# rajgandhi1/threecrate

Measured on AMD Instinct MI355X. Metric: ICP iterations/sec (whole job: k=16 normals + 50-iter point-to-plane ICP per 1M-pt pair; tc_cloud handles, inputs resident in HBM), higher is better.
Workload: dtype f32; 1 GPU; 1000000-pt uniform-random cloud, k=16 normals + 50-iter point-to-plane ICP, independent sigma = 0.0001 noise on source and target, correspondences returned (BASELINE configs[1]; one independent pair per GPU); points=1000000, k=16, parallelism=pairs1, interface=tc_cloud handles (one index build per cloud)

## Files before the change

threecrate_amd/csrc/api.hip:

```cpp
#include "tc_internal.h"
#include <sched.h>
#include <time.h>

#include <algorithm>
#include <cmath>
#include <cstdlib>
#include <cstring>
#include <memory>

namespace tc {

[[maybe_unused]] constexpr int kDebugPrintOnlyBits = 8 | 64 | 256 | 1024;
int debug_flags() {
    static const int flags = [] {
        const char *e = getenv("TC_DEBUG");
        const int f = e ? atoi(e) : 0;
#ifdef TC_DEV
        return f;
#else
        return f & kDebugPrintOnlyBits;
#endif
    }();
    return flags;
}
// ... 67 lines not shown
        for (auto &pb : ctx->pool) (void)hipFree(pb.p);
        ctx->pool.clear(); ctx->pool_bytes = 0;
        e = hipMalloc(&b.p, want);
    }
    if (e != hipSuccess) {
        b.p = nullptr;
        return fail(ctx, TC_GPU, std::string("hipMalloc(") + std::to_string(want) + "): " + hipGetErrorString(e));
    }
    b.cap = want;
    return TC_OK;
}

ProfScope::ProfScope(tc_context *c, const char *name, bool dominant) : ctx(c) {
    if (ctx->profiling != 1 && ctx->profiling != 2) return;
    if (ctx->profiling == 2 && (!dominant || (ctx->prof_tick++ % 37u) != 0)) return;
    for (size_t i = 0; i < ctx->timers.size(); ++i)
        if (ctx->timers[i].name == name) { idx = (int)i; break; }
    if (idx < 0) { ctx->timers.push_back(KernelTimer{name, {}, 0, 0.0, 1e300, 0.0}); idx = (int)ctx->timers.size() - 1; }
    auto get = [&]() {
        hipEvent_t e = nullptr;
        if (!ctx->event_pool.empty()) { e = ctx->event_pool.back(); ctx->event_pool.pop_back(); }
        else (void)hipEventCreate(&e);
        return e;
    };
    e0 = get(); e1 = get();
    ext = dominant;
    if (!ext) (void)hipEventRecord(e0, ctx->stream);
}
ProfScope::~ProfScope() {
    if (idx < 0) return;
    if (!ext) (void)hipEventRecord(e1, ctx->stream);
    ctx->timers[idx].pending.emplace_back(e0, e1);
}

bool pinned_poll_enabled() {
    const char *e = getenv("TC_NO_PINNED_POLL");
    return !(e && atoi(e) != 0);
}

void *pinned_dev_ptr(tc_context *ctx, const void *host_addr) {
    if (!ctx->pinned_dev) {
        void *d = nullptr;
        if (hipHostGetDevicePointer(&d, ctx->pinned, 0) != hipSuccess) return nullptr;
        ctx->pinned_dev = d;
    }
    return (char *)ctx->pinned_dev + ((const char *)host_addr - (const char *)ctx->pinned);
}

static inline void cpu_relax() {
#if defined(__x86_64__) || defined(__i386__)
    __builtin_ia32_pause();
#elif defined(__aarch64__)
    asm volatile("yield" ::: "memory");
#else
    sched_yield();
#endif
}

tc_status wait_pinned_word(tc_context *ctx, volatile uint32_t *word, const char *what) {
    struct timespec t0 = {0, 0};
    bool sleeping = false;
    for (unsigned spins = 0; *word == 0u; ++spins) {
        if (sleeping || (spins & 1023u) == 1023u) {
            const hipError_t q = hipStreamQuery(ctx->stream);
            if (q == hipSuccess) { if (*word == 0u) return fail(ctx, TC_GPU, std::string("internal error: ") + what + ": the stream drained without the word being written"); break; }
            if (q != hipErrorNotReady) return fail(ctx, TC_GPU, std::string(what) + ": " + hipGetErrorString(q));
            if (!sleeping && spins >= 4096u) {
                struct timespec t;
                clock_gettime(CLOCK_MONOTONIC, &t);
                if (t0.tv_sec == 0 && t0.tv_nsec == 0) t0 = t;
                sleeping = (t.tv_sec - t0.tv_sec) * 1000000000ll + (t.tv_nsec - t0.tv_nsec) > 2000000ll;
            }
        }
        if (sleeping) { const struct timespec d = {0, 50000}; nanosleep(&d, nullptr); }
        else if (spins > 4096u) sched_yield();
        else cpu_relax();
    }
    __atomic_thread_fence(__ATOMIC_ACQUIRE);
    return TC_OK;
}

void free_buf(DevBuf &b) { if (b.p) (void)hipFree(b.p); b.p = nullptr; b.cap = 0; }

tc_status upload_async(tc_context *ctx, void *d_dst, const void *h_src, size_t bytes) {
    if (bytes < ((size_t)8 << 20)) {
        TC_HIP_TRY(ctx, hipMemcpyAsync(d_dst, h_src, bytes, hipMemcpyHostToDevice, ctx->stream));
        return TC_OK;
    }
    ctx->upload_used_copy_stream = true;
    if (!ctx->copy_stream) TC_HIP_TRY(ctx, hipStreamCreateWithFlags(&ctx->copy_stream, hipStreamNonBlocking));
    if (!ctx->upload_event) TC_HIP_TRY(ctx, hipEventCreateWithFlags(&ctx->upload_event, hipEventDisableTiming));
    TC_HIP_TRY(ctx, hipMemcpyAsync(d_dst, h_src, bytes, hipMemcpyHostToDevice, ctx->copy_stream));
    return TC_OK;
}
tc_status uploads_issued(tc_context *ctx) {
    if (!ctx->upload_used_copy_stream) return TC_OK;
    ctx->upload_used_copy_stream = false;
    TC_HIP_TRY(ctx, hipEventRecord(ctx->upload_event, ctx->copy_stream));
    ctx->upload_pending = true;
    return TC_OK;
}
tc_status wait_uploads(tc_context *ctx) {
    if (!ctx->upload_pending) return TC_OK;
    ctx->upload_pending = false;
    TC_HIP_TRY(ctx, hipStreamWaitEvent(ctx->stream, ctx->upload_event, 0));
    return TC_OK;
}

tc_status stage_in(tc_context *ctx, DevBuf &b, const void *h_src, size_t bytes) {
    if (tc_status s = ensure(ctx, b, bytes)) return s;
    TC_HIP_TRY(ctx, hipMemcpyAsync(b.p, h_src, bytes, hipMemcpyHostToDevice, ctx->stream));
    return TC_OK;
}

tc_status synced(tc_context *ctx) {
    TC_HIP_TRY(ctx, hipStreamSynchronize(ctx->stream));
    return TC_OK;
}
tc_status stage_out(tc_context *ctx, void *h_dst, const void *d_src, size_t bytes) {
    TC_HIP_TRY(ctx, hipMemcpyAsync(h_dst, d_src, bytes, hipMemcpyDeviceToHost, ctx->stream));
    return synced(ctx);
}
tc_status read_back(tc_context *ctx, void *host_dst, const void *dev_src, size_t bytes) {
    if (tc_status s = stage_out(ctx, host_dst, dev_src, bytes)) return s;
    TC_HIP_TRY(ctx, hipGetLastError());
    return TC_OK;
}

float normals_cell_factor(size_t k, bool large) {
    const double K1 = (double)k + 1.0;
    const double lam = K1 + 3.1 * std::sqrt(K1) + 2.0;
    const double c = std::cbrt(lam / 4.18879);
    return (float)((large ? 1.03 : 0.95) * c / 2.0);
}

float normals_target_ppo(size_t k) {
    const double K1 = (double)k + 1.0;
    return (float)((K1 + 3.1 * std::sqrt(K1) + 2.0) / 11.3);
}

IndexSpec knn_grid(size_t list_len) {
    IndexSpec spec; spec.cell_factor = normals_cell_factor(list_len > 1 ? list_len - 1 : 1, false) * 2.0f;
    return spec;
}
IndexSpec ball_grid(float radius, bool finite_only) {
    const float r2 = radius * radius;
    IndexSpec spec; spec.cell_factor = 0.5f;
    if (r2 <= r2 && (!finite_only || r2 <= 3.0e38f)) { spec.min_cell_edge = 0.5f * radius; spec.target_ppo = 2.0f; }
    return spec;
}

void recycle_index(tc_context *ctx, DeviceIndex &ix) {
    for_each_buf(ix, [ctx](DevBuf &b) { recycle(ctx, b); });
    ix.pts12_valid = false; ix.vor_valid = false;
}

void free_index(DeviceIndex &ix) { for_each_buf(ix, free_buf); }

tc_status normals_on_index(tc_context *ctx, DeviceIndex &ix, bool build, float cell_factor_override, const float *d_xyz, size_t n,
                           const tc_normal_config *cfg, float *d_out, size_t p_begin, size_t p_end, bool slice_out, float4 *d_sorted_nrm,
                           bool with_bounds) {
    if (build) {
        const float min_h = cfg->has_radius ? cfg->radius * 0.5005f : 0.0f;
        const float f = cell_factor_override > 0.0f ? cell_factor_override : normals_cell_factor(cfg->k_neighbors, n >= kAdaptMinPoints);
        IndexSpec spec; spec.cell_factor = f; spec.min_cell_edge = min_h; spec.target_ppo = normals_target_ppo(cfg->k_neighbors); spec.strict_order = slice_out;
        if (tc_status s = build_index(ctx, ix, d_xyz, n, spec)) return s;
    }
    float vp[3];
    if (cfg->has_viewpoint) {
        vp[0] = cfg->viewpoint[0]; vp[1] = cfg->viewpoint[1]; vp[2] = cfg->viewpoint[2];
    } else {
        const float *bmn = ix.exact_min, *bmx = ix.exact_max;
        const float cx = (bmn[0] + bmx[0]) / 2.0f, cy = (bmn[1] + bmx[1]) / 2.0f, cz = (bmn[2] + bmx[2]) / 2.0f;
        const float ex = bmx[0] - bmn[0], ey = bmx[1] - bmn[1], ez = bmx[2] - bmn[2];
        const float extent = std::sqrt(ex * ex + ey * ey + ez * ez);
        vp[0] = cx + 0.0f; vp[1] = cy + 0.0f; vp[2] = cz + extent;
    }
    float4 *d_vor = nullptr;
    const bool knn_mode = !(cfg->has_radius && cfg->radius > 0.0f);
    if (with_bounds && knn_mode && p_begin == 0 && p_end >= n) {
        if (tc_status s = ensure(ctx, ix.vor, n * sizeof(float4))) return s;
        d_vor = (float4 *)ix.vor.p;
    }
    if (tc_status s = launch_normals(ctx, ix, d_xyz, *cfg, vp, d_out, p_begin, p_end, slice_out, d_sorted_nrm, d_vor)) return s;
    ix.vor_valid = d_vor != nullptr;
    return TC_OK;
}

static tc_status normals_device(tc_context *ctx, const float *d_xyz, size_t n, const tc_normal_config *cfg, float *d_out,
                                size_t p_begin = 0, size_t p_end = (size_t)-1, bool slice_out = false) {
    return normals_on_index(ctx, ctx->tgt_index, true, 0.0f, d_xyz, n, cfg, d_out, p_begin, p_end, slice_out, nullptr);
}

}

using namespace tc;

extern "C" {

int tc_abi_version(void) { return TC_ABI_VERSION; }

int tc_device_count(void) try {
    int n = 0;
    if (hipGetDeviceCount(&n) != hipSuccess) return 0;
    return n;
} TC_CATCH_VALUE(0)

static tc_status context_create(int device, void *stream, bool own, tc_context **out) {
    if (!out) return TC_INVALID_DATA;
    *out = nullptr;
    fault_point("context");
    int n = 0;
    if (hipGetDeviceCount(&n) != hipSuccess || n <= 0 || device < 0 || device >= n) return TC_GPU;
    if (hipSetDevice(device) != hipSuccess) return TC_GPU;
    std::unique_ptr<tc_context> holder(new tc_context());
    tc_context *ctx = holder.get();
    ctx->last_error.reserve(256);
    ctx->device = device;
    ctx->own_stream = own;
    if (own) {
        if (hipStreamCreateWithFlags(&ctx->stream, hipStreamNonBlocking) != hipSuccess) return TC_GPU;
    } else {
        ctx->stream = (hipStream_t)stream;
    }
    if (hipHostMalloc(&ctx->pinned, kPinnedBytes, hipHostMallocDefault) != hipSuccess) {
        if (own) (void)hipStreamDestroy(ctx->stream);
        return TC_GPU;
    }
    *out = holder.release();
    return TC_OK;
}

tc_status tc_context_create(int device, tc_context **out) try { return context_create(device, nullptr, true, out); } TC_CATCH_STATUS(nullptr)
tc_status tc_context_create_on_stream(int device, void *hip_stream, tc_context **out) try {
    return context_create(device, hip_stream, false, out);
} TC_CATCH_STATUS(nullptr)

tc_status tc_context_wait_stream(tc_context *ctx, void *other_hip_stream) try {
    if (!ctx) return TC_INVALID_DATA;
    hipStream_t other = (hipStream_t)other_hip_stream;
    if (other == ctx->stream) return TC_OK;
    TC_HIP_TRY(ctx, hipSetDevice(ctx->device));
    if (!ctx->order_event) TC_HIP_TRY(ctx, hipEventCreateWithFlags(&ctx->order_event, hipEventDisableTiming));
    TC_HIP_TRY(ctx, hipEventRecord(ctx->order_event, other));
    TC_HIP_TRY(ctx, hipStreamWaitEvent(ctx->stream, ctx->order_event, 0));
    return TC_OK;
} TC_CATCH_STATUS(ctx)

tc_status tc_stream_wait_context(tc_context *ctx, void *other_hip_stream) try {
    if (!ctx) return TC_INVALID_DATA;
    hipStream_t other = (hipStream_t)other_hip_stream;
    if (other == ctx->stream) return TC_OK;
    TC_HIP_TRY(ctx, hipSetDevice(ctx->device));
    if (!ctx->release_event) TC_HIP_TRY(ctx, hipEventCreateWithFlags(&ctx->release_event, hipEventDisableTiming));
    TC_HIP_TRY(ctx, hipEventRecord(ctx->release_event, ctx->stream));
    TC_HIP_TRY(ctx, hipStreamWaitEvent(other, ctx->release_event, 0));
    return TC_OK;
} TC_CATCH_STATUS(ctx)

void tc_context_destroy(tc_context *ctx) try {
    if (!ctx) return;
    (void)hipSetDevice(ctx->device);
    (void)hipStreamSynchronize(ctx->stream);
    if (ctx->copy_stream) { (void)hipStreamSynchronize(ctx->copy_stream); (void)hipStreamDestroy(ctx->copy_stream); }
    if (ctx->upload_event) (void)hipEventDestroy(ctx->upload_event);
    for_each_buf(*ctx, free_buf);
    for (auto &pb : ctx->pool) (void)hipFree(pb.p);
    for (auto e : ctx->chunk_events) (void)hipEventDestroy(e);
    if (ctx->order_event) (void)hipEventDestroy(ctx->order_event);
    if (ctx->release_event) (void)hipEventDestroy(ctx->release_event);
    for (auto &t : ctx->timers) for (auto &p : t.pending) { (void)hipEventDestroy(p.first); (void)hipEventDestroy(p.second); }
    for (auto e : ctx->event_pool) (void)hipEventDestroy(e);
    if (ctx->pinned) (void)hipHostFree(ctx->pinned);
    if (ctx->own_stream && ctx->stream) (void)hipStreamDestroy(ctx->stream);
    delete ctx;
} TC_CATCH_VOID

tc_status tc_context_trim(tc_context *ctx) try {
    if (!ctx) return TC_INVALID_DATA;
    TC_HIP_TRY(ctx, hipSetDevice(ctx->device));
    TC_HIP_TRY(ctx, hipStreamSynchronize(ctx->stream));
    for (auto &pb : ctx->pool) (void)hipFree(pb.p);
    ctx->pool.clear();
    ctx->pool_bytes = 0;
    ctx->pool_largest = 0;
    return TC_OK;
} TC_CATCH_STATUS(ctx)

const char *tc_last_error_message(const tc_context *ctx) { return ctx ? ctx->last_error.c_str() : "null context"; }

tc_status tc_synchronize(tc_context *ctx) try {
    if (!ctx) return TC_INVALID_DATA;
    return synced(ctx);
} TC_CATCH_STATUS(ctx)

void tc_normal_config_default(tc_normal_config *cfg) try {
    if (!cfg) return;
    std::memset(cfg, 0, sizeof(*cfg));
    cfg->k_neighbors = 10;
    cfg->has_radius = 0;
    cfg->consistent_orientation = 1;
    cfg->has_viewpoint = 0;
} TC_CATCH_VOID

static tc_status normals_validate(tc_context *ctx, size_t n, const tc_normal_config *cfg, bool *empty) {
    *empty = false;
    if (!ctx || !cfg) return TC_INVALID_DATA;
// ... 156 lines not shown
```

threecrate_amd/csrc/cloud.hip:

```cpp
#include "tc_internal.h"

#include <algorithm>
#include <cmath>
#include <cstring>

struct tc_cloud {
    tc_context *ctx = nullptr;
    size_t n = 0;
    tc::DevBuf xyz;
    tc::DeviceIndex ix;
    bool indexed = false;
    float factor = 0.0f;
    bool has_normals = false;
    tc::DevBuf normals6;
    bool has_normals6 = false;
};

namespace {

using namespace tc;


float shared_factor(float want) {
    return (want > 0.8f * kIcpCellFactor && want < 1.25f * kIcpCellFactor) ? kIcpCellFactor : want;
}

__global__ void __launch_bounds__(256) cloud_unsort_normals_kernel(const float4 *__restrict__ pts, const float4 *__restrict__ sorted_nrm,
                                                                  const float *__restrict__ xyz, uint32_t n, float *__restrict__ out6) {
    const uint32_t p = blockIdx.x * blockDim.x + threadIdx.x;
    if (p >= n) return;
    const uint32_t orig = __float_as_uint(pts[p].w);
    const float4 nr = sorted_nrm[p];
    float *o = out6 + 6 * (size_t)orig;
    o[0] = xyz[3 * (size_t)orig]; o[1] = xyz[3 * (size_t)orig + 1]; o[2] = xyz[3 * (size_t)orig + 2];
    o[3] = nr.x; o[4] = nr.y; o[5] = nr.z;
}

tc_status ensure_index(tc_cloud *c, float want_factor, float target_ppo, float min_h) {
    tc_context *ctx = c->ctx;
    const float f = shared_factor(want_factor);
    if (c->indexed && c->factor > 0.8f * f && c->factor < 1.25f * f && min_h <= c->ix.geom.h) return TC_OK;
    if (c->has_normals && !c->has_normals6 && c->indexed && c->n) {
        if (tc_status s = ensure(ctx, c->normals6, c->n * 6 * sizeof(float))) return s;
        hipLaunchKernelGGL(cloud_unsort_normals_kernel, dim3((unsigned)((c->n + 255) / 256)), dim3(256), 0, ctx->stream,
                           (const float4 *)c->ix.pts.p, (const float4 *)c->ix.normals.p, (const float *)c->xyz.p, (uint32_t)c->n,
                           (float *)c->normals6.p);
        TC_HIP_TRY(ctx, hipGetLastError());
        c->has_normals6 = true;
    }
    c->has_normals = false;
    IndexSpec spec; spec.cell_factor = f; spec.min_cell_edge = min_h; spec.target_ppo = target_ppo;
    if (tc_status s = build_index(ctx, c->ix, (const float *)c->xyz.p, c->n, spec)) return s;
    c->indexed = true;
    c->factor = f;
    return TC_OK;
}

tc_status cloud_create(tc_context *ctx, const float *p, size_t n, bool from_host, tc_cloud **out) {
    if (!ctx || !out) return TC_INVALID_DATA;
    *out = nullptr;
    if (tc_status s = check_point_count(ctx, n)) return s;
    TC_HIP_TRY(ctx, hipSetDevice(ctx->device));
    tc_cloud *c = new tc_cloud();
    c->ctx = ctx;
    c->n = n;
    if (n) {
        tc_status s = ensure(ctx, c->xyz, n * 3 * sizeof(float));
        if (s == TC_OK && hipMemcpyAsync(c->xyz.p, p, n * 3 * sizeof(float), from_host ? hipMemcpyHostToDevice : hipMemcpyDeviceToDevice,
                                         ctx->stream) != hipSuccess) s = fail(ctx, TC_GPU, "cloud upload failed");
        if (s == TC_OK && from_host && hipStreamSynchronize(ctx->stream) != hipSuccess) s = fail(ctx, TC_GPU, "cloud upload failed");
        if (s != TC_OK) { recycle(ctx, c->xyz); delete c; return s; }
    }
    *out = c;
    return TC_OK;
}

tc_status adopt_normals(tc_cloud *c, const float *d_normals, size_t stride) {
    if (tc_status s = ensure_index(c, kIcpCellFactor, 2.5f, 0.0f)) return s;
    if (tc_status s = gather_normals(c->ctx, c->ix, d_normals, stride)) return s;
    c->has_normals = true;
    return TC_OK;
}

tc_status prepare_target(tc_cloud *tgt, bool p2plane);

tc_status cloud_icp(tc_cloud *src, tc_cloud *tgt, bool p2plane, const float init[7], size_t max_iters, float max_dist, float conv_thr,
                    tc_icp_result *res) {
    if (!src || !tgt || !res || !init) return TC_INVALID_DATA;
    tc_context *ctx = tgt->ctx;
    if (src->ctx != ctx) return fail(ctx, TC_INVALID_DATA, "source and target handles belong to different contexts");
    if (src->n == 0 || tgt->n == 0) return fail(ctx, TC_INVALID_DATA, "Source or target point cloud is empty");
    if (p2plane && !tgt->has_normals && !tgt->has_normals6)
        return fail(ctx, TC_INVALID_DATA, "target_normals length must equal the number of target points (the target handle has no normals: "
                                          "tc_cloud_estimate_normals or tc_cloud_set_normals_device first)");
    if (max_iters == 0) return fail(ctx, TC_INVALID_DATA, "Max iterations must be positive");
    TC_HIP_TRY(ctx, hipSetDevice(ctx->device));
    if (tc_status s = prepare_target(tgt, p2plane)) return s;
    IcpJob job;
    job.mode = p2plane ? 1 : 0;
    job.src = (const float *)src->xyz.p; job.ns = src->n; job.tgt = (const float *)tgt->xyz.p; job.nt = tgt->n;
    job.init = init; job.max_iters = max_iters; job.max_dist = max_dist; job.conv_thr = conv_thr;
    job.tgt_prebuilt = &tgt->ix;
    job.src_presorted = (src->indexed && src != tgt) ? &src->ix : nullptr;
    return icp_run(ctx, job, res);
}

tc_status prepare_target(tc_cloud *tgt, bool p2plane) {
    tc_context *ctx = tgt->ctx;
    if (tc_status s = ensure_index(tgt, kIcpCellFactor, 2.5f, 0.0f)) return s;
    if (p2plane && !tgt->has_normals) {
        if (!tgt->has_normals6) return fail(ctx, TC_INVALID_DATA, "the target handle has no normals in input order to re-sort after its index was rebuilt");
        if (tc_status s = gather_normals(ctx, tgt->ix, (const float *)tgt->normals6.p + 3, 6)) return s;
        tgt->has_normals = true;
    }
    return TC_OK;
}

}

extern "C" {

tc_status tc_cloud_sharded_icp(tc_comm *comm, int shard_mode, int point_to_plane, const float *d_source, size_t n_source, tc_cloud *target,
                               const float init[7], size_t max_iters, float max_dist, float conv_thr, tc_icp_result *result) try {
    if (!comm || !target || !result || !init) return TC_INVALID_DATA;
    tc_context *ctx = target->ctx;
    if (comm->ctx != ctx) return fail(ctx, TC_INVALID_DATA, "the communicator belongs to another context");
    if (shard_mode != TC_SHARD_SPATIAL && shard_mode != TC_SHARD_LOCAL && shard_mode != TC_SHARD_INDEX) return fail(ctx, TC_INVALID_DATA, "unknown shard mode");
    const bool may_be_empty = shard_mode == TC_SHARD_LOCAL && comm->nranks > 1;
    if ((n_source == 0 && !may_be_empty) || target->n == 0) return fail(ctx, TC_INVALID_DATA, "Source or target point cloud is empty");
    if (point_to_plane && !target->has_normals && !target->has_normals6)
        return fail(ctx, TC_INVALID_DATA, "target_normals length must equal the number of target points (the target handle has no normals)");
    if (max_iters == 0) return fail(ctx, TC_INVALID_DATA, "Max iterations must be positive");
    TC_HIP_TRY(ctx, hipSetDevice(ctx->device));
    if (tc_status s = prepare_target(target, point_to_plane != 0)) return s;
    IcpJob job;
    job.mode = point_to_plane ? 1 : 0;
    job.src = d_source; job.ns = n_source; job.tgt = (const float *)target->xyz.p; job.nt = target->n;
    job.init = init; job.max_iters = max_iters; job.max_dist = max_dist; job.conv_thr = conv_thr;
    job.tgt_prebuilt = &target->ix;
    return icp_run_sharded(ctx, comm, shard_mode, job, result);
} TC_CATCH_STATUS((comm ? comm->ctx : nullptr))

tc_status tc_cloud_upload(tc_context *ctx, const float *xyz, size_t n, tc_cloud **out) try { return cloud_create(ctx, xyz, n, true, out); } TC_CATCH_STATUS(ctx)
tc_status tc_cloud_upload_device(tc_context *ctx, const float *d_xyz, size_t n, tc_cloud **out) try { return cloud_create(ctx, d_xyz, n, false, out); } TC_CATCH_STATUS(ctx)
size_t tc_cloud_size(const tc_cloud *c) { return c ? c->n : 0; }
const float *tc_cloud_points_device(const tc_cloud *c) { return c ? (const float *)c->xyz.p : nullptr; }
const float *tc_cloud_normals_device(const tc_cloud *cc) try {
    tc_cloud *c = const_cast<tc_cloud *>(cc);
    if (!c || c->n == 0) return nullptr;
    if (c->has_normals6) return (const float *)c->normals6.p;
    if (!c->has_normals || !c->indexed) return nullptr;
    tc_context *ctx = c->ctx;
    if (hipSetDevice(ctx->device) != hipSuccess) { (void)fail(ctx, TC_GPU, "tc_cloud_normals_device: hipSetDevice failed"); return nullptr; }
    if (ensure(ctx, c->normals6, c->n * 6 * sizeof(float)) != TC_OK) return nullptr;
    hipLaunchKernelGGL(cloud_unsort_normals_kernel, dim3((unsigned)((c->n + 255) / 256)), dim3(256), 0, ctx->stream,
                       (const float4 *)c->ix.pts.p, (const float4 *)c->ix.normals.p, (const float *)c->xyz.p, (uint32_t)c->n,
                       (float *)c->normals6.p);
    hipError_t e = hipGetLastError();
    if (e == hipSuccess) e = hipStreamSynchronize(ctx->stream);
    if (e != hipSuccess) { (void)fail(ctx, TC_GPU, std::string("tc_cloud_normals_device: ") + hipGetErrorString(e)); return nullptr; }
    c->has_normals6 = true;
    return (const float *)c->normals6.p;
} TC_CATCH_VALUE(nullptr)

static tc_status cloud_normals(tc_cloud *c, const tc_normal_config *cfg, float *out, bool out_on_host, bool keep6) {
    if (!c || !cfg) return TC_INVALID_DATA;
    tc_context *ctx = c->ctx;
    if (c->n == 0) return TC_OK;
    if (cfg->k_neighbors < 3) return fail(ctx, TC_INVALID_DATA, "k_neighbors must be at least 3");
    TC_HIP_TRY(ctx, hipSetDevice(ctx->device));
    const float min_h = cfg->has_radius ? cfg->radius * 0.5005f : 0.0f;
    c->has_normals = false;
    c->has_normals6 = false;
    if (tc_status s = ensure_index(c, normals_cell_factor(cfg->k_neighbors, c->n >= kAdaptMinPoints), normals_target_ppo(cfg->k_neighbors), min_h)) return s;
    if (tc_status s = ensure(ctx, c->ix.normals, c->n * sizeof(float4))) return s;
    const bool direct = out != nullptr && !out_on_host && !keep6;
    const bool want6 = (out != nullptr || keep6) && !direct;
    float *d_out6 = direct ? out : nullptr;
    if (want6) {
        if (tc_status s = ensure(ctx, c->normals6, c->n * 6 * sizeof(float))) return s;
        d_out6 = (float *)c->normals6.p;
    }
    c->has_normals = false;
    c->has_normals6 = false;
    if (tc_status s = normals_on_index(ctx, c->ix, false, 0.0f, (const float *)c->xyz.p, c->n, cfg, d_out6, 0, (size_t)-1, false,
                                       (float4 *)c->ix.normals.p, true)) return s;
    c->has_normals = true;
    c->has_normals6 = want6;
    if (out && !direct) TC_HIP_TRY(ctx, hipMemcpyAsync(out, d_out6, c->n * 6 * sizeof(float), out_on_host ? hipMemcpyDeviceToHost : hipMemcpyDeviceToDevice, ctx->stream));
    TC_HIP_TRY(ctx, hipStreamSynchronize(ctx->stream));
    return TC_OK;
}

tc_status tc_cloud_estimate_normals(tc_cloud *c, const tc_normal_config *cfg, float *out) try { return cloud_normals(c, cfg, out, true, false); } TC_CATCH_STATUS(c ? c->ctx : nullptr)
tc_status tc_cloud_estimate_normals_device(tc_cloud *c, const tc_normal_config *cfg, float *d_out) try { return cloud_normals(c, cfg, d_out, false, false); } TC_CATCH_STATUS(c ? c->ctx : nullptr)

tc_status tc_cloud_set_normals_device(tc_cloud *c, const float *d_normals, size_t n_normals, size_t stride) try {
    if (!c) return TC_INVALID_DATA;
    tc_context *ctx = c->ctx;
    if (n_normals != c->n) return fail(ctx, TC_INVALID_DATA, "target_normals length must equal the number of target points");
    if (stride < 3) return fail(ctx, TC_INVALID_DATA, "normal_stride must be >= 3");
    if (c->n == 0) return TC_OK;
    TC_HIP_TRY(ctx, hipSetDevice(ctx->device));
    c->has_normals = false;
// ... 27 lines not shown
```

threecrate_amd/csrc/grid.hip:

```cpp
#include "tc_internal.h"
#include <rocprim/device/device_radix_sort.hpp>

#include <algorithm>
#include <cmath>
#include <cstring>

namespace tc {

constexpr int kBboxBlocks = 256;
__device__ __forceinline__ uint32_t f2ord(float f) { const uint32_t b = __float_as_uint(f); return (b & 0x80000000u) ? ~b : (b | 0x80000000u); }
__device__ __forceinline__ float ord2f(uint32_t u) { return __uint_as_float((u & 0x80000000u) ? (u ^ 0x80000000u) : ~u); }
constexpr uint32_t kOrdPlusInf = 0xFF800000u, kOrdMinusInf = 0x007FFFFFu;
constexpr uint32_t kBboxAccStride = 32;
constexpr size_t kBboxStateBytes = 31 * kBboxAccStride * sizeof(uint32_t), kBboxBufBytes = kBboxStateBytes + 128 + 256;

template <bool VEC>
__global__ void __launch_bounds__(256) bbox_kernel(const float *__restrict__ xyz, uint32_t n, uint32_t *__restrict__ state, int robust,
                                                  float *__restrict__ out, uint32_t *__restrict__ done) {
    const bool sbox = robust != 0;
    __shared__ float sm[4][30];
    float v[30];
#pragma unroll
    for (int k = 0; k < 30; ++k) v[k] = (k % 6 < 3) ? INFINITY : -INFINITY;
    auto take = [&](float x, float y, float z, uint32_t i, int s) {
        if (!(fabsf(x) <= 3.0e38f && fabsf(y) <= 3.0e38f && fabsf(z) <= 3.0e38f)) return;
        v[0] = fminf(v[0], x); v[1] = fminf(v[1], y); v[2] = fminf(v[2], z);
        v[3] = fmaxf(v[3], x); v[4] = fmaxf(v[4], y); v[5] = fmaxf(v[5], z);
        if (sbox && ((i * 2654435761u) >> 28) == 0u) {
            float *b = v + 6 + 6 * s;
            b[0] = fminf(b[0], x); b[1] = fminf(b[1], y); b[2] = fminf(b[2], z);
            b[3] = fmaxf(b[3], x); b[4] = fmaxf(b[4], y); b[5] = fmaxf(b[5], z);
        }
    };
    const uint32_t gt = blockIdx.x * blockDim.x + threadIdx.x, stride = gridDim.x * blockDim.x;
    if constexpr (VEC) {
        const float4 *__restrict__ q = reinterpret_cast<const float4 *>(xyz);
        const uint32_t nq = n >> 2;
        constexpr int U = 4;
        for (uint32_t c0 = gt; c0 < nq; c0 += U * stride) {
            float4 a[U], b[U], c[U];
#pragma unroll
            for (int u = 0; u < U; ++u) {
                const uint32_t cc = min(c0 + (uint32_t)u * stride, nq - 1u);
                a[u] = q[3 * (size_t)cc]; b[u] = q[3 * (size_t)cc + 1]; c[u] = q[3 * (size_t)cc + 2];
            }
#pragma unroll
            for (int u = 0; u < U; ++u) {
                const uint32_t i = 4u * min(c0 + (uint32_t)u * stride, nq - 1u);
                take(a[u].x, a[u].y, a[u].z, i, 0);
                take(a[u].w, b[u].x, b[u].y, i + 1u, 1);
                take(b[u].z, b[u].w, c[u].x, i + 2u, 2);
                take(c[u].y, c[u].z, c[u].w, i + 3u, 3);
            }
        }
        if (gt < (n & 3u)) {
            const uint32_t i = (nq << 2) + gt;
            const float x = xyz[3 * (size_t)i], y = xyz[3 * (size_t)i + 1], z = xyz[3 * (size_t)i + 2];
            if ((i & 3u) == 0u) take(x, y, z, i, 0); else if ((i & 3u) == 1u) take(x, y, z, i, 1); else take(x, y, z, i, 2);
        }
    } else {
        for (uint32_t i = gt; i < n; i += stride) {
            const float x = xyz[3 * (size_t)i], y = xyz[3 * (size_t)i + 1], z = xyz[3 * (size_t)i + 2];
            const uint32_t sidx = threadIdx.x & 3u;
            if (sidx == 0u) take(x, y, z, i, 0); else if (sidx == 1u) take(x, y, z, i, 1); else if (sidx == 2u) take(x, y, z, i, 2); else take(x, y, z, i, 3);
        }
    }
#pragma unroll
    for (int k = 0; k < 30; ++k) {
        if (k < 6 || sbox) {
#pragma unroll
            for (int o = 32; o > 0; o >>= 1) {
                const float w = __shfl_xor(v[k], o);
                v[k] = (k % 6 < 3) ? fminf(v[k], w) : fmaxf(v[k], w);
            }
        }
    }
    if ((threadIdx.x & 63) == 0) {
#pragma unroll
        for (int k = 0; k < 30; ++k) sm[threadIdx.x >> 6][k] = v[k];
    }
    __syncthreads();
    uint32_t *acc = state + kBboxAccStride;
    if (threadIdx.x < (sbox ? 30 : 6)) {
        const bool is_min = threadIdx.x % 6 < 3;
        float r = sm[0][threadIdx.x];
        for (int w = 1; w < 4; ++w) r = is_min ? fminf(r, sm[w][threadIdx.x]) : fmaxf(r, sm[w][threadIdx.x]);
        if (is_min) atomicMin(&acc[threadIdx.x * kBboxAccStride], f2ord(r)); else atomicMax(&acc[threadIdx.x * kBboxAccStride], f2ord(r));
    }
    __shared__ uint32_t s_last;
    if (threadIdx.x < 64) {
        asm volatile("s_waitcnt vmcnt(0)" ::: "memory");
        if (threadIdx.x == 0) s_last = __hip_atomic_fetch_add(state, 1u, __ATOMIC_RELAXED, __HIP_MEMORY_SCOPE_AGENT) == gridDim.x - 1u ? 1u : 0u;
    }
    __syncthreads();
    if (!s_last) return;
    if (threadIdx.x < 30) {
        const uint32_t u = __hip_atomic_load(&acc[threadIdx.x * kBboxAccStride], __ATOMIC_RELAXED, __HIP_MEMORY_SCOPE_AGENT);
        __hip_atomic_store(&out[threadIdx.x], ord2f(u), __ATOMIC_RELAXED, __HIP_MEMORY_SCOPE_SYSTEM);
        __hip_atomic_store(&acc[threadIdx.x * kBboxAccStride], (threadIdx.x % 6 < 3) ? kOrdPlusInf : kOrdMinusInf, __ATOMIC_RELAXED, __HIP_MEMORY_SCOPE_AGENT);
    }
    if (threadIdx.x == 0) __hip_atomic_store(state, 0u, __ATOMIC_RELAXED, __HIP_MEMORY_SCOPE_AGENT);
    if (done) {
        if (threadIdx.x < 30) __threadfence_system();
        __syncthreads();
        if (threadIdx.x == 0) __hip_atomic_store(done, 1u, __ATOMIC_RELEASE, __HIP_MEMORY_SCOPE_SYSTEM);
    }
}

__global__ void bbox_state_init_kernel(uint32_t *__restrict__ state) {
    const uint32_t t = threadIdx.x;
    if (t == 0) state[0] = 0u;
    if (t < 30) state[(t + 1) * kBboxAccStride] = (t % 6 < 3) ? kOrdPlusInf : kOrdMinusInf;
}


__global__ void __launch_bounds__(256) cell_hist_kernel(const float *__restrict__ xyz, uint32_t n, GridGeom g,
                                                       const IcpState *__restrict__ st, TileGeom tg, int tile_major, uint32_t nkeys,
                                                       uint32_t *__restrict__ cell_of, uint32_t *__restrict__ hist,
                                                       uint32_t *__restrict__ arrival, uint32_t *__restrict__ pts_pad,
                                                       uint32_t *__restrict__ cs_front, uint32_t *__restrict__ cs_tail, uint32_t rank_max) {
    uint32_t i = blockIdx.x * blockDim.x + threadIdx.x;
    if (blockIdx.x == 0 && threadIdx.x < 4 * kPtsPad + kCellStartFront + kCellStartPad) {
        const uint32_t t = threadIdx.x;
        if (t < 4 * kPtsPad) pts_pad[t] = 0x7F7F7F7Fu;
        else if (t < 4 * kPtsPad + kCellStartFront) cs_front[t - 4 * kPtsPad] = 0u;
        else cs_tail[t - 4 * kPtsPad - kCellStartFront] = 0u;
    }
    if (i >= n) return;
    float x = xyz[3 * (size_t)i], y = xyz[3 * (size_t)i + 1], z = xyz[3 * (size_t)i + 2];
    if (st) {
        float q[4] = {st->q[0], st->q[1], st->q[2], st->q[3]}, t[3] = {st->t[0], st->t[1], st->t[2]};
        float ox, oy, oz;
        isometry_apply(q, t, x, y, z, ox, oy, oz);
        x = ox; y = oy; z = oz;
    }
    int ix = cell_coord(x, g.minx, g.inv_h, g.gx);
    int iy = cell_coord(y, g.miny, g.inv_h, g.gy);
    int iz = cell_coord(z, g.minz, g.inv_h, g.gz);
    uint32_t c = tile_major ? tile_major_id(tg, ix, iy, iz) : ((uint32_t)iz * g.gy + iy) * g.gx + ix;
    if (!(fabsf(x) <= 3.0e38f && fabsf(y) <= 3.0e38f && fabsf(z) <= 3.0e38f)) c = nkeys;
    cell_of[i] = c;
    const uint32_t a = atomicAdd(&hist[c], 1u);
    arrival[i] = a;
    if (a == rank_max) hist[nkeys + 1] = 1u;
}

__global__ void __launch_bounds__(256) iota_kernel(uint32_t *__restrict__ p, uint32_t n) {
    const uint32_t i = blockIdx.x * blockDim.x + threadIdx.x;
    if (i < n) p[i] = i;
}

constexpr int kScanItems = 8;
constexpr int kScanBlock = 256;
constexpr int kScanTile = kScanItems * kScanBlock;

__global__ void __launch_bounds__(kScanBlock) scan_reduce_kernel(const uint32_t *__restrict__ in, uint32_t n,
                                                                 uint32_t *__restrict__ blocksum) {
    __shared__ uint32_t wsum[kScanBlock / 64], wnz[kScanBlock / 64];
    uint32_t base = blockIdx.x * kScanTile;
    uint32_t s = 0, nz = 0;
#pragma unroll
    for (int k = 0; k < kScanItems; ++k) {
        uint32_t i = base + k * kScanBlock + threadIdx.x;
        if (i < n) { const uint32_t v = in[i]; s += v; nz += v != 0; }
    }
#pragma unroll
    for (int o = 32; o > 0; o >>= 1) { s += __shfl_xor(s, o); nz += __shfl_xor(nz, o); }
    if ((threadIdx.x & 63) == 0) { wsum[threadIdx.x >> 6] = s; wnz[threadIdx.x >> 6] = nz; }
    __syncthreads();
    if (threadIdx.x == 0) {
        blocksum[blockIdx.x] = wsum[0] + wsum[1] + wsum[2] + wsum[3];
        blocksum[gridDim.x + blockIdx.x] = wnz[0] + wnz[1] + wnz[2] + wnz[3];
    }
}

constexpr uint32_t kScanFusedMax = 2048;
__global__ void __launch_bounds__(1024) scan_top_kernel(uint32_t *__restrict__ blocksum, uint32_t nb) {
    __shared__ uint32_t wtot[16];
    uint32_t carry = 0;
    for (uint32_t base = 0; base < nb; base += 1024) {
        const uint32_t i = base + threadIdx.x;
        const uint32_t v = i < nb ? blocksum[i] : 0u;
        uint32_t inc = v;
#pragma unroll
        for (int o = 1; o < 64; o <<= 1) {
            const uint32_t t = __shfl_up(inc, o);
            if ((threadIdx.x & 63) >= (unsigned)o) inc += t;
        }
        if ((threadIdx.x & 63) == 63) wtot[threadIdx.x >> 6] = inc;
        __syncthreads();
        uint32_t woff = 0, tot = 0;
        for (int w = 0; w < 16; ++w) { if (w < (int)(threadIdx.x >> 6)) woff += wtot[w]; tot += wtot[w]; }
        if (i < nb) blocksum[i] = carry + woff + inc - v;
        carry += tot;
        __syncthreads();
    }
}

__global__ void __launch_bounds__(kScanBlock) scan_apply_kernel(const uint32_t *__restrict__ in, uint32_t n,
                                                                uint32_t *__restrict__ blocksum,
                                                                uint32_t *__restrict__ out , uint32_t *__restrict__ occ_out, int prefixed,
                                                                unsigned long long *__restrict__ occ_host) {
    __shared__ uint32_t wtot[kScanBlock / 64];
    __shared__ uint32_t wpre[kScanBlock / 64], wnz[kScanBlock / 64];
    uint32_t pre = 0, nzt = 0;
    if (prefixed) { if (threadIdx.x == 0) pre = blocksum[blockIdx.x]; }
    else for (uint32_t i = threadIdx.x; i < blockIdx.x; i += kScanBlock) pre += blocksum[i];
    if (blockIdx.x == 0) for (uint32_t i = threadIdx.x; i < gridDim.x; i += kScanBlock) nzt += blocksum[gridDim.x + i];
#pragma unroll
    for (int o = 32; o > 0; o >>= 1) { pre += __shfl_xor(pre, o); nzt += __shfl_xor(nzt, o); }
    if ((threadIdx.x & 63) == 0) { wpre[threadIdx.x >> 6] = pre; wnz[threadIdx.x >> 6] = nzt; }
    uint32_t base = blockIdx.x * kScanTile + threadIdx.x * kScanItems;
    uint32_t v[kScanItems];
    uint32_t s = 0;
#pragma unroll
    for (int k = 0; k < kScanItems; ++k) {
        uint32_t i = base + k;
        v[k] = (i < n) ? in[i] : 0;
        s += v[k];
    }
    uint32_t inc = s;
#pragma unroll
    for (int o = 1; o < 64; o <<= 1) {
        uint32_t t = __shfl_up(inc, o);
        if ((threadIdx.x & 63) >= (unsigned)o) inc += t;
    }
    if ((threadIdx.x & 63) == 63) wtot[threadIdx.x >> 6] = inc;
    __syncthreads();
    uint32_t woff = 0;
    for (int w = 0; w < (int)(threadIdx.x >> 6); ++w) woff += wtot[w];
    uint32_t block_pre = 0;
    for (int w = 0; w < kScanBlock / 64; ++w) block_pre += wpre[w];
    if (blockIdx.x == 0 && threadIdx.x == 0) {
        uint32_t t = 0;
        for (int w = 0; w < kScanBlock / 64; ++w) t += wnz[w];
        blocksum[2 * gridDim.x] = t;
        if (occ_out) *occ_out = t;
        if (occ_host) __hip_atomic_store(occ_host, (1ull << 32) | (unsigned long long)t, __ATOMIC_RELAXED, __HIP_MEMORY_SCOPE_SYSTEM);
    }
    uint32_t run = block_pre + woff + inc - s;
#pragma unroll
    for (int k = 0; k < kScanItems; ++k) {
        uint32_t i = base + k;
        if (i < n) out[i] = run;
        run += v[k];
        if (i == n - 1) out[n] = run;
    }
}

__global__ void __launch_bounds__(256) rank_gather_kernel(const float *__restrict__ xyz, uint32_t n, uint32_t nkeys,
                                                         const uint32_t *__restrict__ cell_of,
                                                         const uint32_t *__restrict__ cell_start,
                                                         const uint32_t *__restrict__ slot,
                                                         float4 *__restrict__ pts, int slot_is_ordered, uint32_t rank_max) {
    uint32_t p = blockIdx.x * blockDim.x + threadIdx.x;
    if (p >= n) return;
    uint32_t i = slot[p];
    uint32_t c = cell_of[i];
    uint32_t s = cell_start[c], e = cell_start[c + 1];
    uint32_t rank;
    if (slot_is_ordered) {
        rank = p - s;
    } else if (e - s <= rank_max) {
        rank = 0;
        for (uint32_t j = s; j < e; ++j) rank += (slot[j] < i) ? 1u : 0u;
    } else {
        rank = p - s;
    }
    float4 r;
    r.x = xyz[3 * (size_t)i]; r.y = xyz[3 * (size_t)i + 1]; r.z = xyz[3 * (size_t)i + 2];
    if (c == nkeys) r.x = r.y = r.z = __uint_as_float(0x7F7F7F7Fu);
    r.w = __uint_as_float(i);
    pts[s + rank] = r;
}

__global__ void __launch_bounds__(256) place_kernel(const float *__restrict__ xyz, uint32_t n, uint32_t nkeys,
                                                   const uint32_t *__restrict__ cell_of, const uint32_t *__restrict__ cell_start,
                                                   const uint32_t *__restrict__ arrival, float4 *__restrict__ tmp) {
    const uint32_t i = blockIdx.x * blockDim.x + threadIdx.x;
    if (i >= n) return;
    const uint32_t c = cell_of[i];
    const uint32_t pos = cell_start[c] + arrival[i];
    float4 r;
    r.x = xyz[3 * (size_t)i]; r.y = xyz[3 * (size_t)i + 1]; r.z = xyz[3 * (size_t)i + 2];
    if (c == nkeys) r.x = r.y = r.z = __uint_as_float(0x7F7F7F7Fu);
    r.w = __uint_as_float(i);
    tmp[pos] = r;
}

__global__ void __launch_bounds__(256) rerank_kernel(uint32_t n, GridGeom g, const IcpState *__restrict__ st, TileGeom tg, int tile_major,
                                                    uint32_t nkeys, const uint32_t *__restrict__ cell_start, const float4 *__restrict__ tmp,
                                                    float4 *__restrict__ pts, uint32_t rank_max) {
    const uint32_t p = blockIdx.x * blockDim.x + threadIdx.x;
    if (p >= n) return;
    const float4 r = tmp[p];
    uint32_t c;
    {
        float x = r.x, y = r.y, z = r.z;
        if (st) {
            float q[4] = {st->q[0], st->q[1], st->q[2], st->q[3]}, t[3] = {st->t[0], st->t[1], st->t[2]};
            float ox, oy, oz;
            isometry_apply(q, t, x, y, z, ox, oy, oz);
            x = ox; y = oy; z = oz;
        }
        const int ix = cell_coord(x, g.minx, g.inv_h, g.gx), iy = cell_coord(y, g.miny, g.inv_h, g.gy), iz = cell_coord(z, g.minz, g.inv_h, g.gz);
        c = tile_major ? tile_major_id(tg, ix, iy, iz) : ((uint32_t)iz * g.gy + iy) * g.gx + ix;
        if (!(fabsf(x) <= 3.0e38f && fabsf(y) <= 3.0e38f && fabsf(z) <= 3.0e38f)) c = nkeys;
    }
    const uint32_t s = cell_start[c], e = cell_start[c + 1];
    const uint32_t i = __float_as_uint(r.w);
    uint32_t rank;
    if (e - s <= rank_max) {
        rank = 0;
#pragma unroll 4
        for (uint32_t j = s; j < e; ++j) rank += (__float_as_uint(tmp[j].w) < i) ? 1u : 0u;
    } else {
        rank = p - s;
    }
    pts[s + rank] = r;
}

__global__ void __launch_bounds__(256) gather_normals_kernel(const float4 *__restrict__ pts, uint32_t n,
                                                            const float *__restrict__ nrm, size_t stride,
                                                            float4 *__restrict__ out) {
    uint32_t p = blockIdx.x * blockDim.x + threadIdx.x;
    if (p >= n) return;
    uint32_t i = __float_as_uint(pts[p].w);
    const float *s = nrm + (size_t)i * stride;
    out[p] = make_float4(s[0], s[1], s[2], 0.0f);
}

GridView view_of(const DeviceIndex &ix) {
    GridView v;
    v.g = ix.geom;
    v.pts = (const float4 *)ix.pts.p;
    v.cell_start = (const uint32_t *)ix.cell_start.p + kCellStartFront;
    v.pts12 = ix.pts12_valid ? (const float *)ix.pts12.p : nullptr;
    return v;
}

static void set_cell_edge(GridGeom &g, double h, size_t n, double cells_per_point) {
    const double e[3] = {(double)g.maxx - g.minx, (double)g.maxy - g.miny, (double)g.maxz - g.minz};
    const double max_cells = std::max<double>(cells_per_point * (double)n, 4096.0);
    for (int guard = 0; guard < 200; ++guard) {
        double gx = std::floor(e[0] / h) + 1.0, gy = std::floor(e[1] / h) + 1.0, gz = std::floor(e[2] / h) + 1.0;
        if (gx * gy * gz <= max_cells && gx * gy * gz < 2.0e9) {
            g.gx = (int)gx; g.gy = (int)gy; g.gz = (int)gz;
            break;
        }
        h *= 1.2;
    }
    g.h = (float)h;
    g.inv_h = 1.0f / g.h;
    g.ncell = (uint32_t)g.gx * (uint32_t)g.gy * (uint32_t)g.gz;
    g.n = (uint32_t)n;
}

static void derive_geom(GridGeom &g, const float mn[3], const float mx[3], size_t n, float f, float min_h) {
    g.minx = mn[0]; g.miny = mn[1]; g.minz = mn[2];
    g.maxx = mx[0]; g.maxy = mx[1]; g.maxz = mx[2];
    g.cx = 0.5f * (mn[0] + mx[0]); g.cy = 0.5f * (mn[1] + mx[1]); g.cz = 0.5f * (mn[2] + mx[2]);
    double e[3] = {(double)mx[0] - mn[0], (double)mx[1] - mn[1], (double)mx[2] - mn[2]};
    double emax = std::max(e[0], std::max(e[1], e[2]));
    double h = 1.0;
    if (!(emax > 0.0) || !std::isfinite(emax)) {
        h = 1.0;
    } else {
        double measure = 1.0;
        int dims = 0;
        for (int a = 0; a < 3; ++a)
            if (e[a] > 1e-6 * emax) { measure *= e[a]; ++dims; }
        h = f * std::pow(measure / (double)std::max<size_t>(n, 1), 1.0 / (double)dims);
        if (!(h > 0.0) || !std::isfinite(h)) h = emax;
        h = std::max(h, emax * 1e-4);
    }
    if (min_h > 0.0f && std::isfinite(min_h)) h = std::max(h, (double)min_h);
    set_cell_edge(g, h, n, 8.0);
}

TileGeom make_tiles(const GridGeom &g, int tx, int ty, int tz) {
    TileGeom t;
    t.tx = std::max(tx, 1); t.ty = std::max(ty, 1); t.tz = std::max(tz, 1);
    t.ntx = (g.gx + t.tx - 1) / t.tx; t.nty = (g.gy + t.ty - 1) / t.ty; t.ntz = (g.gz + t.tz - 1) / t.tz;
    t.cpt = (uint32_t)(t.tx * t.ty * t.tz);
    t.ntiles = (uint32_t)t.ntx * (uint32_t)t.nty * (uint32_t)t.ntz;
    return t;
}

tc_status exclusive_scan_u32(tc_context *ctx, const uint32_t *d_in, uint32_t n, uint32_t *d_out, DevBuf &blocksum, uint32_t *occ_out,
                             unsigned long long *occ_host) {
    hipStream_t st = ctx->stream;
    const uint32_t nscan = (n + kScanTile - 1) / kScanTile;
    if (tc_status s = ensure(ctx, blocksum, ((size_t)2 * nscan + 1) * sizeof(uint32_t))) return s;
    hipLaunchKernelGGL(scan_reduce_kernel, dim3(nscan), dim3(kScanBlock), 0, st, d_in, n, (uint32_t *)blocksum.p);
    const char *fm = getenv("TC_SCAN_FUSED_MAX");
    const bool prefixed = nscan > (fm ? (uint32_t)atoi(fm) : kScanFusedMax);
    if (prefixed) hipLaunchKernelGGL(scan_top_kernel, dim3(1), dim3(1024), 0, st, (uint32_t *)blocksum.p, nscan);
    hipLaunchKernelGGL(scan_apply_kernel, dim3(nscan), dim3(kScanBlock), 0, st, d_in, n, (uint32_t *)blocksum.p, d_out, occ_out, prefixed ? 1 : 0, occ_host);
    TC_HIP_TRY(ctx, hipGetLastError());
    return TC_OK;
}

__global__ void __launch_bounds__(256) compact_flagged_kernel(const float *__restrict__ xyz, uint32_t n, const uint32_t *__restrict__ flag,
                                                             const uint32_t *__restrict__ pos, float *__restrict__ out_xyz, uint32_t *__restrict__ out_index) {
    const uint32_t i = blockIdx.x * blockDim.x + threadIdx.x;
    if (i >= n || !flag[i]) return;
    store_compacted(xyz, i, pos[i], out_xyz, out_index);
}

tc_status compact_flagged(tc_context *ctx, const float *d_xyz, uint32_t n, const uint32_t *d_flag, uint32_t *d_pos, DevBuf &blocksum, float *d_out_xyz,
                          uint32_t *d_out_index) {
    if (tc_status s = exclusive_scan_u32(ctx, d_flag, n, d_pos, blocksum)) return s;
    hipLaunchKernelGGL(compact_flagged_kernel, dim3((n + 255u) / 256u), dim3(256), 0, ctx->stream, d_xyz, n, d_flag, (const uint32_t *)d_pos, d_out_xyz, d_out_index);
    return TC_OK;
}

unsigned bits_for_value(uint64_t v) {
    unsigned b = 1;
    while (b < 64 && (1ull << b) <= v) ++b;
    return b;
}

template <class K>
tc_status sort_pairs(tc_context *ctx, const K *keys, K *keys_out, const uint32_t *vals, uint32_t *vals_out, size_t n, unsigned end_bit, DevBuf &temp) {
    K *k_in = const_cast<K *>(keys);
    uint32_t *v_in = const_cast<uint32_t *>(vals);
    size_t temp_bytes = 0;
    TC_HIP_TRY(ctx, rocprim::radix_sort_pairs(nullptr, temp_bytes, k_in, keys_out, v_in, vals_out, n, 0u, end_bit, ctx->stream));
    if (tc_status s = ensure(ctx, temp, temp_bytes)) return s;
    TC_HIP_TRY(ctx, rocprim::radix_sort_pairs(temp.p, temp_bytes, k_in, keys_out, v_in, vals_out, n, 0u, end_bit, ctx->stream));
    return TC_OK;
}
template tc_status sort_pairs<uint64_t>(tc_context *, const uint64_t *, uint64_t *, const uint32_t *, uint32_t *, size_t, unsigned, DevBuf &);
template tc_status sort_pairs<uint32_t>(tc_context *, const uint32_t *, uint32_t *, const uint32_t *, uint32_t *, size_t, unsigned, DevBuf &);

__global__ void __launch_bounds__(256) key_head_kernel(const uint64_t *__restrict__ keys, uint32_t n, uint32_t *__restrict__ head) {
    const uint32_t p = blockIdx.x * blockDim.x + threadIdx.x;
    if (p >= n) return;
    head[p] = (p == 0 || keys[p] != keys[p - 1]) ? 1u : 0u;
}

__global__ void __launch_bounds__(256) key_starts_kernel(uint32_t n, const uint32_t *__restrict__ head, const uint32_t *__restrict__ runpos,
                                                         uint32_t *__restrict__ rstart) {
    const uint32_t p = blockIdx.x * blockDim.x + threadIdx.x;
    if (p >= n) return;
    if (head[p]) rstart[runpos[p]] = p;
    if (p == n - 1) rstart[runpos[n]] = n;
}

tc_status key_runs(tc_context *ctx, const uint64_t *keys_sorted, uint32_t n, uint32_t *head, uint32_t *runpos, uint32_t *rstart, DevBuf &blocksum) {
    const dim3 grid((n + 255u) / 256u), block(256);
    hipLaunchKernelGGL(key_head_kernel, grid, block, 0, ctx->stream, keys_sorted, n, head);
    if (tc_status s = exclusive_scan_u32(ctx, head, n, runpos, blocksum)) return s;
    hipLaunchKernelGGL(key_starts_kernel, grid, block, 0, ctx->stream, n, (const uint32_t *)head, (const uint32_t *)runpos, rstart);
    return TC_OK;
}

tc_status group_by_key(tc_context *ctx, const uint64_t *keys, const uint32_t *vals, size_t n, unsigned key_bits, const GroupBufs &b, KeyGroups &g, size_t room) {
    const size_t items = std::max(n, room);
    const std::pair<DevBuf *, size_t> need[] = {{&b.keys_sorted, items * sizeof(uint64_t)}, {&b.vals_sorted, items * sizeof(uint32_t)},
                                                {&b.head, items * sizeof(uint32_t)}, {&b.runpos, (items + 1) * sizeof(uint32_t)},
                                                {&b.rstart, (items + 1) * sizeof(uint32_t)}};
    for (const auto &[buf, bytes] : need) if (tc_status s = ensure(ctx, *buf, bytes)) return s;
    uint64_t *keys_sorted = (uint64_t *)b.keys_sorted.p;
    uint32_t *order = (uint32_t *)b.vals_sorted.p, *head = (uint32_t *)b.head.p, *runpos = (uint32_t *)b.runpos.p, *rstart = (uint32_t *)b.rstart.p;
    g = KeyGroups{keys_sorted, order, head, runpos, rstart, runpos + n};
    if (tc_status s = sort_pairs(ctx, keys, keys_sorted, vals, order, n, key_bits, b.sort_temp)) return s;
    return key_runs(ctx, keys_sorted, (uint32_t)n, head, runpos, rstart, b.blocksum);
}

static tc_status cloud_bbox_impl(tc_context *ctx, const float *d_xyz, size_t n, float mn[3], float mx[3], float *rmn, float *rmx,
                                 bool *clamped) {
    hipStream_t st = ctx->stream;
    const int nb = (int)((n + 255) / 256);
    const int bb = std::min(nb, kBboxBlocks);
    const bool robust = rmn != nullptr && n >= 4096;
    const bool poll = pinned_poll_enabled();
    const bool fresh = ctx->bbox.p == nullptr;
    if (tc_status s = ensure(ctx, ctx->bbox, kBboxBufBytes)) return s;
    uint32_t *d_state = (uint32_t *)ctx->bbox.p;
    if (fresh) hipLaunchKernelGGL(bbox_state_init_kernel, dim3(1), dim3(64), 0, st, d_state);
    float *hb = pinned_host(ctx)->bbox;
    volatile uint32_t *h_done = &pinned_host(ctx)->bbox_done;
    float *d_out = (float *)((char *)ctx->bbox.p + kBboxStateBytes + 128);
    uint32_t *d_done = nullptr;
    if (poll) {
        d_out = (float *)pinned_dev_ptr(ctx, hb);
        d_done = (uint32_t *)pinned_dev_ptr(ctx, (const void *)h_done);
        if (!d_out || !d_done) return fail(ctx, TC_GPU, "bbox: the pinned block has no device address");
        *h_done = 0u;
    }
    {
        ProfScope ps(ctx, "bbox");
        if (((uintptr_t)d_xyz & 15u) == 0u)
            hipLaunchKernelGGL(bbox_kernel<true>, dim3(std::min((int)((n / 4 + 255) / 256) + 1, kBboxBlocks)), dim3(256), 0, st, d_xyz, (uint32_t)n, d_state, robust ? 1 : 0, d_out, d_done);
        else
            hipLaunchKernelGGL(bbox_kernel<false>, dim3(bb), dim3(256), 0, st, d_xyz, (uint32_t)n, d_state, robust ? 1 : 0, d_out, d_done);
    }
    TC_HIP_TRY(ctx, hipGetLastError());
    if (poll) {
        if (tc_status s = wait_pinned_word(ctx, h_done, "bounding box")) { hipLaunchKernelGGL(bbox_state_init_kernel, dim3(1), dim3(64), 0, st, d_state); return s; }
    } else {
        TC_HIP_TRY(ctx, hipMemcpyAsync(hb, d_out, 30 * sizeof(float), hipMemcpyDeviceToHost, st));
        TC_HIP_TRY(ctx, hipStreamSynchronize(st));
    }
    const float *hs = hb + 6;
    for (int c = 0; c < 3; ++c) { mn[c] = INFINITY; mx[c] = -INFINITY; }
    for (int c = 0; c < 3; ++c) { mn[c] = std::fmin(mn[c], hb[c]); mx[c] = std::fmax(mx[c], hb[3 + c]); }
    if (rmn) {
        for (int c = 0; c < 3; ++c) { rmn[c] = mn[c]; rmx[c] = mx[c]; }
        *clamped = false;
    }
    if (!robust) return TC_OK;
    float acc[24];
    for (int i = 0; i < 24; ++i) acc[i] = (i % 6 < 3) ? INFINITY : -INFINITY;
    for (int i = 0; i < 24; ++i) acc[i] = (i % 6 < 3) ? (hs[i] < acc[i] ? hs[i] : acc[i]) : (hs[i] > acc[i] ? hs[i] : acc[i]);
    for (int c = 0; c < 3; ++c) {
        float lo[4], hi[4];
        for (int k = 0; k < 4; ++k) { lo[k] = acc[6 * k + c]; hi[k] = acc[6 * k + 3 + c]; }
        std::sort(lo, lo + 4);
        std::sort(hi, hi + 4, [](float a, float b) { return a > b; });
        const float slo = lo[2], shi = hi[2];
        if (!(slo <= shi) || !std::isfinite(slo) || !std::isfinite(shi)) continue;
        const float ext = shi - slo, full = mx[c] - mn[c];
        if (!(full > 1.3f * ext) || !(full > 0.0f)) continue;
        rmn[c] = std::fmax(mn[c], slo - 0.05f * ext);
        rmx[c] = std::fmin(mx[c], shi + 0.05f * ext);
        *clamped = true;
    }
    return TC_OK;
}

tc_status cloud_bbox(tc_context *ctx, const float *d_xyz, size_t n, float mn[3], float mx[3]) {
    return cloud_bbox_impl(ctx, d_xyz, n, mn, mx, nullptr, nullptr, nullptr);
}


constexpr int kBinBlocks = 256;
constexpr int kBinWalkThreads = 1024;
#ifndef TC_BIN_TARGET
#define TC_BIN_TARGET 2048
#endif
#ifndef TC_BIN_PLACE_THREADS
#define TC_BIN_PLACE_THREADS 512
#endif
constexpr uint32_t kBinTarget = TC_BIN_TARGET;
constexpr uint32_t kBinCap = 2 * kBinTarget;
constexpr uint32_t kBinKeysMax = 2 * kBinTarget;
static_assert((kBinKeysMax + 3 * kBinCap) * sizeof(uint32_t) + 256 <= 160 * 1024, "bin_place_kernel's static LDS exceeds a gfx950 CU's 160 KB");
#if defined(__HIP_DEVICE_COMPILE__) && !defined(__gfx950__)
#error "libthreecrate_hip is written for gfx950 (MI355X): bin_place_kernel alone needs more than 64 KB of LDS per workgroup"
#endif
constexpr uint32_t kBinMaxBins = 8192;
constexpr int kBinPlaceThreads = TC_BIN_PLACE_THREADS;

__device__ __forceinline__ uint32_t point_key(float x, float y, float z, const GridGeom &g, const IcpState *__restrict__ st, const TileGeom &tg,
                                              int tile_major, uint32_t nkeys) {
    if (st) {
        float q[4] = {st->q[0], st->q[1], st->q[2], st->q[3]}, t[3] = {st->t[0], st->t[1], st->t[2]};
        float ox, oy, oz;
        isometry_apply(q, t, x, y, z, ox, oy, oz);
        x = ox; y = oy; z = oz;
    }
    const int ix = cell_coord(x, g.minx, g.inv_h, g.gx), iy = cell_coord(y, g.miny, g.inv_h, g.gy), iz = cell_coord(z, g.minz, g.inv_h, g.gz);
    uint32_t c = tile_major ? tile_major_id(tg, ix, iy, iz) : ((uint32_t)iz * g.gy + iy) * g.gx + ix;
    if (!(fabsf(x) <= 3.0e38f && fabsf(y) <= 3.0e38f && fabsf(z) <= 3.0e38f)) c = nkeys;
    return c;
}

__global__ void __launch_bounds__(kBinWalkThreads) bin_count_kernel(const float *__restrict__ xyz, uint32_t n, GridGeom g, const IcpState *__restrict__ st,
                                                       TileGeom tg, int tile_major, uint32_t nkeys, uint32_t kpb, uint32_t nbins,
                                                       uint32_t *__restrict__ cnt , uint32_t *__restrict__ pts_pad,
                                                       uint32_t *__restrict__ cs_front, uint32_t *__restrict__ cs_tail) {
    __shared__ uint32_t c[kBinMaxBins];
    if (blockIdx.x == 0 && threadIdx.x < 4 * kPtsPad + kCellStartFront + kCellStartPad) {
        const uint32_t t = threadIdx.x;
        if (t < 4 * kPtsPad) pts_pad[t] = 0x7F7F7F7Fu;
        else if (t < 4 * kPtsPad + kCellStartFront) cs_front[t - 4 * kPtsPad] = 0u;
        else cs_tail[t - 4 * kPtsPad - kCellStartFront] = 0u;
    }
    for (uint32_t b = threadIdx.x; b < nbins; b += kBinWalkThreads) c[b] = 0u;
    __syncthreads();
    const uint32_t per = (n + kBinBlocks - 1) / kBinBlocks;
    const uint32_t i0 = blockIdx.x * per, i1 = min(i0 + per, n);
    for (uint32_t i = i0 + threadIdx.x; i < i1; i += kBinWalkThreads) {
        const uint32_t k = point_key(xyz[3 * (size_t)i], xyz[3 * (size_t)i + 1], xyz[3 * (size_t)i + 2], g, st, tg, tile_major, nkeys);
        atomicAdd(&c[min(k / kpb, nbins - 1u)], 1u);
    }
    __syncthreads();
    for (uint32_t b = threadIdx.x; b < nbins; b += kBinWalkThreads) cnt[(size_t)b * kBinBlocks + blockIdx.x] = c[b];
}

static_assert(kBinBlocks == 256, "one wave x four entries per lane");
__global__ void __launch_bounds__(256) bin_offsets_kernel(uint32_t *__restrict__ cnt, uint32_t nbins, uint32_t *__restrict__ tot) {
    const uint32_t b = blockIdx.x * 4u + (threadIdx.x >> 6), lane = threadIdx.x & 63u;
    if (b >= nbins) return;
    uint4 *row = reinterpret_cast<uint4 *>(cnt + (size_t)b * kBinBlocks);
    const uint4 v = row[lane];
    const uint32_t s = v.x + v.y + v.z + v.w;
    uint32_t inc = s;
#pragma unroll
    for (int o = 1; o < 64; o <<= 1) {
        const uint32_t t = __shfl_up(inc, o);
        if (lane >= (unsigned)o) inc += t;
    }
    const uint32_t ex = inc - s;
    row[lane] = make_uint4(ex, ex + v.x, ex + v.x + v.y, ex + v.x + v.y + v.z);
    if (lane == 63u) tot[b] = inc;
}

__global__ void __launch_bounds__(kBinWalkThreads) bin_scatter_kernel(const float *__restrict__ xyz, uint32_t n, GridGeom g, const IcpState *__restrict__ st,
                                                         TileGeom tg, int tile_major, uint32_t nkeys, uint32_t kpb, uint32_t nbins,
                                                         const uint32_t *__restrict__ off ,
                                                         const uint32_t *__restrict__ tot, uint32_t *__restrict__ binstart,
                                                         uint32_t *__restrict__ occ_ticket, unsigned long long *__restrict__ host_word,
                                                         float4 *__restrict__ tmp) {
    static_assert(kBinWalkThreads == 1024, "the scan below is written for 16 waves");
    __shared__ uint32_t cur[kBinMaxBins];
    __shared__ uint32_t wtot[16], wmax[16];
    uint32_t carry = 0, mx = 0;
    for (uint32_t base = 0; base < nbins; base += kBinWalkThreads) {
        const uint32_t i = base + threadIdx.x;
        const uint32_t v = i < nbins ? tot[i] : 0u;
        const uint32_t o_mine = i < nbins ? off[(size_t)i * kBinBlocks + blockIdx.x] : 0u;
        mx = max(mx, v);
        uint32_t inc = v;
#pragma unroll
        for (int o = 1; o < 64; o <<= 1) {
            const uint32_t t = __shfl_up(inc, o);
            if ((threadIdx.x & 63) >= (unsigned)o) inc += t;
        }
        if ((threadIdx.x & 63) == 63) wtot[threadIdx.x >> 6] = inc;
        __syncthreads();
        uint32_t woff = 0, total = 0;
        for (int w = 0; w < 16; ++w) { if (w < (int)(threadIdx.x >> 6)) woff += wtot[w]; total += wtot[w]; }
        const uint32_t start = carry + woff + inc - v;
        if (i < nbins) {
            cur[i] = start + o_mine;
            if (blockIdx.x == 0) binstart[i] = start;
        }
        carry += total;
        __syncthreads();
    }
    if (blockIdx.x == 0) {
#pragma unroll
        for (int o = 32; o > 0; o >>= 1) mx = max(mx, (uint32_t)__shfl_xor(mx, o));
        if ((threadIdx.x & 63) == 0) wmax[threadIdx.x >> 6] = mx;
        __syncthreads();
        if (threadIdx.x == 0) {
            binstart[nbins] = carry;
            uint32_t m = 0;
            for (int w = 0; w < 16; ++w) m = max(m, wmax[w]);
            occ_ticket[0] = 0u; occ_ticket[1] = 0u;
            occ_ticket[2] = m;
            __hip_atomic_store(host_word, (1ull << 32) | (unsigned long long)m, __ATOMIC_RELAXED, __HIP_MEMORY_SCOPE_SYSTEM);
        }
    }
    const uint32_t per = (n + kBinBlocks - 1) / kBinBlocks;
    const uint32_t i0 = blockIdx.x * per, i1 = min(i0 + per, n);
    for (uint32_t i = i0 + threadIdx.x; i < i1; i += kBinWalkThreads) {
        float4 r;
        r.x = xyz[3 * (size_t)i]; r.y = xyz[3 * (size_t)i + 1]; r.z = xyz[3 * (size_t)i + 2];
        const uint32_t k = point_key(r.x, r.y, r.z, g, st, tg, tile_major, nkeys);
        if (k == nkeys) r.x = r.y = r.z = __uint_as_float(0x7F7F7F7Fu);
        r.w = __uint_as_float(i);
        tmp[atomicAdd(&cur[min(k / kpb, nbins - 1u)], 1u)] = r;
    }
}

__global__ void __launch_bounds__(kBinPlaceThreads) bin_place_kernel(const float4 *__restrict__ tmp, const uint32_t *__restrict__ binstart,
                                                                     uint32_t nbins, uint32_t kpb, uint32_t nkeys, GridGeom g,
                                                                     const IcpState *__restrict__ st, TileGeom tg, int tile_major,
                                                                     uint32_t *__restrict__ cs, float4 *__restrict__ pts,
                                                                     uint32_t *__restrict__ occ_ticket, uint32_t *__restrict__ occ_out,
                                                                     unsigned long long *__restrict__ occ_host) {
    __shared__ uint32_t cnt[kBinKeysMax];
    __shared__ uint32_t rkey[kBinCap];
    __shared__ uint32_t ridx[kBinCap];
    __shared__ uint32_t slot[kBinCap];
    __shared__ uint32_t wsum[kBinPlaceThreads / 64];
    __shared__ uint32_t s_occ;
    const uint32_t bin = blockIdx.x, tid = threadIdx.x;
    if (occ_ticket[2] > kBinCap) return;
    const uint32_t bs = binstart[bin], P = binstart[bin + 1] - bs;
    const uint32_t k0 = bin * kpb, K = min(kpb, nkeys + 1u - k0);
    for (uint32_t k = tid; k < K; k += kBinPlaceThreads) cnt[k] = 0u;
    if (tid == 0) s_occ = 0u;
    __syncthreads();
    for (uint32_t i = tid; i < P; i += kBinPlaceThreads) {
        const float4 r = tmp[bs + i];
        const uint32_t k = min(point_key(r.x, r.y, r.z, g, st, tg, tile_major, nkeys) - k0, K - 1u);
        const uint32_t a = atomicAdd(&cnt[k], 1u);
        rkey[i] = k | (a << 16);
        ridx[i] = __float_as_uint(r.w);
    }
    __syncthreads();
    constexpr uint32_t kPer = kBinKeysMax / kBinPlaceThreads;
    uint32_t v[kPer], sum = 0, nz = 0;
#pragma unroll
    for (uint32_t t = 0; t < kPer; ++t) {
        const uint32_t k = tid * kPer + t;
        v[t] = k < K ? cnt[k] : 0u;
        sum += v[t];
        nz += v[t] != 0u;
    }
    uint32_t inc = sum;
#pragma unroll
    for (int o = 1; o < 64; o <<= 1) {
        const uint32_t t2 = __shfl_up(inc, o);
        if ((tid & 63) >= (unsigned)o) inc += t2;
    }
#pragma unroll
    for (int o = 32; o > 0; o >>= 1) nz += __shfl_xor(nz, o);
    if ((tid & 63) == 63) wsum[tid >> 6] = inc;
    if ((tid & 63) == 0 && nz) atomicAdd(&s_occ, nz);
    __syncthreads();
    uint32_t run = inc - sum;
    for (uint32_t w = 0; w < (tid >> 6); ++w) run += wsum[w];
#pragma unroll
    for (uint32_t t = 0; t < kPer; ++t) {
        const uint32_t k = tid * kPer + t;
        if (k < K) { cnt[k] = run; cs[k0 + k] = bs + run; }
        run += v[t];
    }
    if (bin == nbins - 1 && tid == 0) cs[nkeys + 1] = bs + P;
    __syncthreads();
    for (uint32_t i = tid; i < P; i += kBinPlaceThreads) slot[cnt[rkey[i] & 0xFFFFu] + (rkey[i] >> 16)] = ridx[i];
    __syncthreads();
    for (uint32_t i = tid; i < P; i += kBinPlaceThreads) {
        const uint32_t k = rkey[i] & 0xFFFFu, me = ridx[i];
        const uint32_t s0 = cnt[k], e0 = (k + 1 < K) ? cnt[k + 1] : P;
        uint32_t rank = 0;
        for (uint32_t j = s0; j < e0; ++j) rank += slot[j] < me ? 1u : 0u;
        rkey[i] = s0 + rank;
    }
    __syncthreads();
    for (uint32_t i = tid; i < P; i += kBinPlaceThreads) slot[rkey[i]] = i;
    __syncthreads();
    for (uint32_t t = tid; t < P; t += kBinPlaceThreads) pts[bs + t] = tmp[bs + slot[t]];
    if (tid == 0) {
        const unsigned long long mine = ((unsigned long long)s_occ << 32) | 1ull;
        const unsigned long long old = __hip_atomic_fetch_add(reinterpret_cast<unsigned long long *>(occ_ticket), mine, __ATOMIC_RELAXED, __HIP_MEMORY_SCOPE_AGENT);
        if ((uint32_t)old == nbins - 1u) {
            const uint32_t occ = (uint32_t)(old >> 32) + s_occ;
            if (occ_out) __hip_atomic_store(occ_out, occ, __ATOMIC_RELAXED, __HIP_MEMORY_SCOPE_AGENT);
            if (occ_host) __hip_atomic_store(occ_host, (1ull << 32) | (unsigned long long)occ, __ATOMIC_RELAXED, __HIP_MEMORY_SCOPE_SYSTEM);
        }
    }
}

static uint32_t rank_quadratic_max() {
    const char *e = getenv("TC_RANK_QUADRATIC_MAX");
    return e ? (uint32_t)std::max(1, atoi(e)) : kRankQuadraticMax;
}

static bool binned_build_enabled() {
    const char *e = getenv("TC_INDEX_BINNED");
    return !(e && atoi(e) == 0);
}

tc_status build_index(tc_context *ctx, DeviceIndex &ix, const float *d_xyz, size_t n, const IndexSpec &spec) {
    if (n == 0 || n >= kMaxPoints) return fail(ctx, TC_INVALID_DATA, "build_index: bad point count");
    ctx->stat_indexed_points += n;
    ctx->stat_index_builds += 1;
    ix.vor_valid = false;
    ix.pts12_valid = false;
    ix.occ_host_valid = false;
    hipStream_t st = ctx->stream;
    const uint32_t n32 = (uint32_t)n;
    const int nb = (int)((n + 255) / 256);
    const int dbg = debug_flags();
    const uint32_t rank_max = rank_quadratic_max();

    if (spec.reuse_geom) {
        ix.geom = *spec.reuse_geom;
        ix.geom.n = n32;
    } else {
        float mn[3], mx[3], rmn[3], rmx[3];
        bool clamped = false;
        if (tc_status s = cloud_bbox_impl(ctx, d_xyz, n, mn, mx, rmn, rmx, &clamped)) return s;
        if (dbg & 2048) clamped = false, std::memcpy(rmn, mn, sizeof(mn)), std::memcpy(rmx, mx, sizeof(mx));
        for (int c = 0; c < 3; ++c) {
            if (!(mn[c] <= mx[c]) || !std::isfinite(mn[c]) || !std::isfinite(mx[c])) { mn[c] = 0.0f; mx[c] = 0.0f; rmn[c] = 0.0f; rmx[c] = 0.0f; }
            ix.exact_min[c] = mn[c]; ix.exact_max[c] = mx[c];
        }
        derive_geom(ix.geom, rmn, rmx, n, spec.cell_factor, spec.min_cell_edge);
        ix.geom.clamped = clamped ? 1 : 0;
        if ((dbg & 256) && clamped)
            fprintf(stderr, "[tc] index: box clamped to %g..%g %g..%g %g..%g (exact %g..%g %g..%g %g..%g)\n", rmn[0], rmx[0], rmn[1], rmx[1],
                    rmn[2], rmx[2], mn[0], mx[0], mn[1], mx[1], mn[2], mx[2]);
    }
    const bool adapt = spec.target_ppo > 0.0f && !spec.reuse_geom && !spec.tile_major && n >= kAdaptMinPoints && !(dbg & 512);
    uint32_t nkeys_final = 0;
    const uint32_t *cs_final = nullptr;
    for (int attempt = 0;; ++attempt) {
        const GridGeom g = ix.geom;
        TileGeom tg{};
        uint32_t nkeys = g.ncell;
        if (spec.tile_major) {
            tg = *spec.tile_major;
            ix.tile = tg;
            const uint64_t nk = (uint64_t)tg.ntiles * tg.cpt;
            if (nk >= kMaxPoints) return fail(ctx, TC_UNSUPPORTED, "tile-major key space too large");
            nkeys = (uint32_t)nk;
        }

        if (tc_status s = ensure(ctx, ix.pts, (n + kPtsPad) * sizeof(float4))) return s;
        if (tc_status s = ensure(ctx, ix.cell_of, n * sizeof(uint32_t))) return s;
        if (tc_status s = ensure(ctx, ix.slot, n * sizeof(uint32_t))) return s;
        if (tc_status s = ensure(ctx, ix.arrival, n * sizeof(uint32_t))) return s;
        const size_t fill_bytes = (((size_t)nkeys + 2) * sizeof(uint32_t) + 255) & ~(size_t)255;
        if (tc_status s = ensure(ctx, ix.fill, fill_bytes)) return s;
        if (tc_status s = ensure(ctx, ix.cell_start, (kCellStartFront + (size_t)nkeys + 2 + kCellStartPad) * sizeof(uint32_t))) return s;
        uint32_t *const cs = (uint32_t *)ix.cell_start.p + kCellStartFront;
        nkeys_final = nkeys; cs_final = cs;
        const bool check = adapt && attempt < 3;
        volatile uint32_t *h_occ = pinned_host(ctx)->occ;

        bool binned_done = false;
        if (binned_build_enabled() && pinned_poll_enabled() && !spec.strict_order && n >= kAdaptMinPoints && n <= (1u << 24) && nkeys < 0x7FFFFFF0u) {
            const uint32_t keys = nkeys + 1u;
            uint32_t nbins = std::max<uint32_t>((n32 + kBinTarget - 1) / kBinTarget, (keys + kBinKeysMax - 1) / kBinKeysMax);
            const uint32_t kpb = (keys + nbins - 1) / nbins;
            nbins = (keys + kpb - 1) / kpb;
            if (nbins <= kBinMaxBins && kpb <= kBinKeysMax) {
                const size_t words = 4 + (size_t)kBinBlocks * nbins + nbins + (nbins + 1);
                if (tc_status s = ensure(ctx, ix.fill, std::max(fill_bytes, words * sizeof(uint32_t)))) return s;
                uint32_t *occ_ticket = (uint32_t *)ix.fill.p, *cnt = occ_ticket + 4, *tot = cnt + (size_t)kBinBlocks * nbins, *binstart = tot + nbins;
                volatile uint32_t *h_max = pinned_host(ctx)->bin_max;
                unsigned long long *d_max = (unsigned long long *)pinned_dev_ptr(ctx, (const void *)h_max);
                if (!d_max) return fail(ctx, TC_GPU, "index build: the pinned block has no device address");
                h_max[0] = 0u; h_max[1] = 0u;
                {
                    ProfScope ps(ctx, "cell_bin_count");
                    hipLaunchKernelGGL(bin_count_kernel, dim3(kBinBlocks), dim3(kBinWalkThreads), 0, st, d_xyz, n32, g, spec.state_transform, tg, spec.tile_major ? 1 : 0, nkeys, kpb,
                                       nbins, cnt, reinterpret_cast<uint32_t *>((float4 *)ix.pts.p + n), (uint32_t *)ix.cell_start.p, cs + nkeys + 2);
                }
                {
                    ProfScope ps(ctx, "cell_bin_offsets");
                    hipLaunchKernelGGL(bin_offsets_kernel, dim3((nbins + 3) / 4), dim3(256), 0, st, cnt, nbins, tot);
                }
                if (tc_status s = ensure(ctx, ctx->build_tmp, (n + kPtsPad) * sizeof(float4))) return s;
                {
                    ProfScope ps(ctx, "cell_bin_scatter");
                    hipLaunchKernelGGL(bin_scatter_kernel, dim3(kBinBlocks), dim3(kBinWalkThreads), 0, st, d_xyz, n32, g, spec.state_transform, tg, spec.tile_major ? 1 : 0, nkeys,
                                       kpb, nbins, (const uint32_t *)cnt, (const uint32_t *)tot, binstart, occ_ticket, d_max, (float4 *)ctx->build_tmp.p);
                }
                if (check) { h_occ[0] = 0u; h_occ[1] = 0u; }
                unsigned long long *d_occ_host = check ? (unsigned long long *)pinned_dev_ptr(ctx, (const void *)h_occ) : nullptr;
                {
                    ProfScope ps(ctx, "cell_bin_place");
                    hipLaunchKernelGGL(bin_place_kernel, dim3(nbins), dim3(kBinPlaceThreads), 0, st, (const float4 *)ctx->build_tmp.p, (const uint32_t *)binstart,
                                       nbins, kpb, nkeys, g, spec.state_transform, tg, spec.tile_major ? 1 : 0, cs, (float4 *)ix.pts.p, occ_ticket,
                                       (uint32_t *)ix.cell_start.p, d_occ_host);
                }
                TC_HIP_TRY(ctx, hipGetLastError());
                if (tc_status s = wait_pinned_word(ctx, h_max + 1, "index build (bin populations)")) return s;
                if (h_max[0] <= kBinCap) {
                    binned_done = true;
                } else if (dbg & 256) {
                    fprintf(stderr, "[tc] index: largest bin holds %u points (> %u): atomic counting sort\n", h_max[0], kBinCap);
                }
            }
        }
        if (!binned_done) {
        TC_HIP_TRY(ctx, hipMemsetAsync(ix.fill.p, 0, fill_bytes, st));
        {
            ProfScope ps(ctx, "cell_hist");
            hipLaunchKernelGGL(cell_hist_kernel, dim3(nb), dim3(256), 0, st, d_xyz, n32, g, spec.state_transform, tg, spec.tile_major ? 1 : 0, nkeys,
                               (uint32_t *)ix.cell_of.p, (uint32_t *)ix.fill.p, (uint32_t *)ix.arrival.p,
                               reinterpret_cast<uint32_t *>((float4 *)ix.pts.p + n), (uint32_t *)ix.cell_start.p, cs + nkeys + 2, rank_max);
        }
        {
            ProfScope ps(ctx, "cell_scan");
            if (check) { h_occ[0] = 0u; h_occ[1] = 0u; }
            unsigned long long *d_occ_host = (check && pinned_poll_enabled()) ? (unsigned long long *)pinned_dev_ptr(ctx, (const void *)h_occ) : nullptr;
            if (check && pinned_poll_enabled() && !d_occ_host) return fail(ctx, TC_GPU, "index build: the pinned block has no device address");
            if (tc_status s = exclusive_scan_u32(ctx, (const uint32_t *)ix.fill.p, nkeys + 1, cs, ix.blocksum, (uint32_t *)ix.cell_start.p, d_occ_host)) return s;
        }
        if (tc_status s = ensure(ctx, ctx->build_tmp, (n + kPtsPad) * sizeof(float4))) return s;
        {
            ProfScope ps(ctx, "cell_place");
            hipLaunchKernelGGL(place_kernel, dim3(nb), dim3(256), 0, st, d_xyz, n32, nkeys, (const uint32_t *)ix.cell_of.p, (const uint32_t *)cs,
                               (const uint32_t *)ix.arrival.p, (float4 *)ctx->build_tmp.p);
        }
        {
            ProfScope ps(ctx, "cell_rerank");
            hipLaunchKernelGGL(rerank_kernel, dim3(nb), dim3(256), 0, st, n32, g, spec.state_transform, tg, spec.tile_major ? 1 : 0, nkeys, (const uint32_t *)cs,
                               (const float4 *)ctx->build_tmp.p, (float4 *)ix.pts.p, rank_max);
        }
        }
        TC_HIP_TRY(ctx, hipGetLastError());
        if (!check) break;
        if (pinned_poll_enabled()) {
            if (tc_status s = wait_pinned_word(ctx, h_occ + 1, "index build (occupied cells)")) return s;
        } else {
            const uint32_t nscan = (nkeys + 1 + kScanTile - 1) / kScanTile;
            TC_HIP_TRY(ctx, hipMemcpyAsync((void *)h_occ, (const uint32_t *)ix.blocksum.p + 2 * nscan, sizeof(uint32_t), hipMemcpyDeviceToHost, st));
            TC_HIP_TRY(ctx, hipStreamSynchronize(st));
        }
        const uint32_t occ_now = h_occ[0];
        const double ppo = (double)n / (double)std::max<uint32_t>(occ_now, 1u);
        ix.occ_host = occ_now; ix.occ_host_valid = true;
        if (dbg & 256)
            fprintf(stderr, "[tc] index: n %zu h %.5f grid %d x %d x %d = %u cells (%.2f n), %u occupied, %.2f points each (want %.1f)\n", n,
                    g.h, g.gx, g.gy, g.gz, g.ncell, (double)g.ncell / (double)n, occ_now, ppo, spec.target_ppo);
        if (!(ppo > 2.0 * spec.target_ppo)) break;
        double h = (double)g.h * std::min(0.8, std::max(0.35, std::sqrt((double)spec.target_ppo / ppo)));
        if (spec.min_cell_edge > 0.0f) h = std::max(h, (double)spec.min_cell_edge);
        GridGeom ng = g;
        set_cell_edge(ng, h, n, 32.0);
        if (!(ng.h < 0.95f * g.h)) break;
        ix.geom = ng;
        ix.occ_host_valid = false;
    }
    if (spec.strict_order) {
        if (tc_status s = read_back(ctx, &pinned_host(ctx)->big_cell, (const uint32_t *)ix.fill.p + nkeys_final + 1, sizeof(uint32_t))) return s;
        if (pinned_host(ctx)->big_cell) {
            if (tc_status s = ensure(ctx, ctx->overflow, n * sizeof(uint32_t))) return s;
            uint32_t *iota = (uint32_t *)ix.arrival.p, *keys_out = (uint32_t *)ctx->overflow.p;
            hipLaunchKernelGGL(iota_kernel, dim3(nb), dim3(256), 0, st, iota, n32);
            if (tc_status s = sort_pairs(ctx, (const uint32_t *)ix.cell_of.p, keys_out, (const uint32_t *)iota, (uint32_t *)ix.slot.p, n,
                                         bits_for_value(nkeys_final), ix.blocksum)) return s;
            ProfScope ps(ctx, "cell_rank_gather_strict");
            hipLaunchKernelGGL(rank_gather_kernel, dim3(nb), dim3(256), 0, st, d_xyz, n32, nkeys_final, (const uint32_t *)ix.cell_of.p,
                               (const uint32_t *)cs_final, (const uint32_t *)ix.slot.p, (float4 *)ix.pts.p, 1, rank_max);
            TC_HIP_TRY(ctx, hipGetLastError());
        }
    }
    return TC_OK;
}

tc_status gather_normals(tc_context *ctx, DeviceIndex &ix, const float *d_normals, size_t stride) {
    const size_t n = ix.geom.n;
    if (tc_status s = ensure(ctx, ix.normals, n * sizeof(float4))) return s;
    ProfScope ps(ctx, "gather_normals");
    hipLaunchKernelGGL(gather_normals_kernel, dim3((unsigned)((n + 255) / 256)), dim3(256), 0, ctx->stream,
                       (const float4 *)ix.pts.p, (uint32_t)n, d_normals, stride, (float4 *)ix.normals.p);
    TC_HIP_TRY(ctx, hipGetLastError());
    return TC_OK;
}

}
```

threecrate_amd/csrc/icp.hip:

```cpp
#include "tc_internal.h"
#include <hip/hip_ext.h>

#include <algorithm>
#include <type_traits>
#include <cmath>
#include <cstring>
#include <cstdlib>
#include <cstdio>

namespace tc {

typedef uint32_t u32x16 __attribute__((ext_vector_type(16)));
struct IcpHeader {
    float q[4], t[3];
    float prev_mse, conv_thr, max_dist;
    uint32_t iterations;
    int32_t done;
    float d_ang, d_t;
    uint32_t d_run;
};
static_assert(offsetof(IcpState, done) == 48 && offsetof(IcpState, max_dist) == 60 && offsetof(IcpState, iterations) == 36 &&
              offsetof(IcpState, prev_mse) == 28 && offsetof(IcpState, conv_thr) == 56, "IcpState header layout");
__device__ __forceinline__ IcpHeader load_header(const IcpState *st) {
    const u32x16 h = *reinterpret_cast<const u32x16 *>(st);
// ... 825 lines not shown
#pragma unroll
    for (int k = 0; k < kCntPer; ++k) {
        const uint32_t b = threadIdx.x * per + k;
        const uint32_t v = rlist[min(b, n_segs - 1)];
        cnt[k] = b < n_segs ? v : 0u;
    }
    if (hd.done) return;
    double folded = 0.0;
#pragma unroll
    for (int k = 0; k < kFoldBatch; ++k) folded += fr[k];
    if (threadIdx.x < TC_ICP_SUMS_STRIDE)
        for (uint32_t r = mr0 + kFoldBatch; r < mr1; ++r) folded += main_rows[(size_t)r * TC_ICP_SUMS_STRIDE + threadIdx.x];
    const GridGeom &g = tgt.g;
    const float q[4] = {hd.q[0], hd.q[1], hd.q[2], hd.q[3]};
    const float max_dist = hd.max_dist;
    __shared__ uint32_t seg_off[kMaxPartialBlocks * kSegPerRow + 1];
    __shared__ uint32_t wave_tot[kRefineThreads / 64];
    {
        uint32_t run = 0;
#pragma unroll
        for (int k = 0; k < kCntPer; ++k) run += cnt[k];
        uint32_t inc = run;
#pragma unroll
        for (int o = 1; o < 64; o <<= 1) {
            const uint32_t v = __shfl_up(inc, o);
            if ((int)(threadIdx.x & 63) >= o) inc += v;
        }
        if ((threadIdx.x & 63) == 63) wave_tot[threadIdx.x >> 6] = inc;
        __syncthreads();
        uint32_t ex = inc - run;
        for (int w2 = 0; w2 < (int)(threadIdx.x >> 6); ++w2) ex += wave_tot[w2];
#pragma unroll
        for (int k = 0; k < kCntPer; ++k) {
            const uint32_t b = threadIdx.x * per + k;
            if (b <= n_segs) seg_off[b] = ex;
            ex += cnt[k];
        }
        if (threadIdx.x == kRefineThreads - 1) seg_off[n_segs] = ex;
        __syncthreads();
    }
    const uint32_t count = seg_off[n_segs];
    const uint4 *__restrict__ entries = refine_entries(rlist);
    if (blockIdx.x == 0 && threadIdx.x == 0) {
        st->refine_total += count;
        st->refine_max = max(st->refine_max, count);
    }
    if ((uint32_t)blockIdx.x >= count) {
        if (threadIdx.x < TC_ICP_SUMS_STRIDE) partial_rows[(size_t)blockIdx.x * TC_ICP_SUMS_STRIDE + threadIdx.x] = folded;
        return;
    }
    const __amdgpu_buffer_rsrc_t pt_rsrc = raw_rsrc(tgt.pts), cs_rsrc = raw_rsrc(tgt.cell_start);
    const int lg = threadIdx.x & (kRG - 1);
    const uint32_t group = (threadIdx.x / kRG) * gridDim.x + blockIdx.x, ngroups = gridDim.x * kRefineThreads / kRG;
    const unsigned long long gmask = (kRG == 64) ? ~0ull : (((1ull << kRG) - 1ull) << ((threadIdx.x & 63) & ~(kRG - 1)));
    float *const acc = lacc[threadIdx.x / kRG];
    for (int k = lg; k < NACC; k += kRG) acc[k] = 0.0f;
    __builtin_amdgcn_fence(__ATOMIC_RELEASE, "wavefront");
    auto locate = [&](uint32_t i) -> size_t {
        uint32_t lo = 0, nleft = n_segs;
        while (nleft > 1) {
            const uint32_t stride = (nleft + kRG - 1) / kRG;
            const bool le = (uint32_t)lg * stride < nleft && seg_off[lo + lg * stride] <= i;
            const uint32_t m = (uint32_t)((__ballot(le) & gmask) >> ((threadIdx.x & 63) & ~(kRG - 1)));
            const uint32_t k = 31u - (uint32_t)__clz((int)m);
            lo += k * stride;
            nleft = min(stride, nleft - k * stride);
        }
        return (size_t)lo * seg_stride + (i - seg_off[lo]);
    };
    uint4 n0 = make_uint4(0, 0, 0, 0), n1 = n0;
    if (group < count) { const size_t a = locate(group); n0 = entries[2 * a]; n1 = entries[2 * a + 1]; }
    for (uint32_t i = group; i < count; i += ngroups) {
        const uint4 e0 = n0, e1 = n1;
        if (i + ngroups < count) { const size_t a = locate(i + ngroups); n0 = entries[2 * a]; n1 = entries[2 * a + 1]; }
        const uint32_t j = e0.w, pj = e1.y;
        const float x = __uint_as_float(e0.x), y = __uint_as_float(e0.y), z = __uint_as_float(e0.z);
        const float qx = fminf(fmaxf(x, g.minx), g.maxx), qy = fminf(fmaxf(y, g.miny), g.maxy),
                    qz = fminf(fmaxf(z, g.minz), g.maxz);
        const int cx = cell_coord(qx, g.minx, g.inv_h, g.gx), cy = cell_coord(qy, g.miny, g.inv_h, g.gy),
                  cz = cell_coord(qz, g.minz, g.inv_h, g.gz);
        const float fx = (qx - g.minx) * g.inv_h - (float)cx, fy = (qy - g.miny) * g.inv_h - (float)cy,
                    fz = (qz - g.minz) * g.inv_h - (float)cz;
        const float out2 = outside_d2(x, y, z, qx, qy, qz, g.clamped);
        unsigned long long bestkey = ~0ull;
        if (pj != 0xFFFFFFFFu) bestkey = ((unsigned long long)e1.x << 32) | pj;
        if (bestkey != ~0ull && !dbg_shells)
            bestkey = refine_ball_scan(tgt, cs_rsrc, pt_rsrc, lg, x, y, z, bestkey, max_dist >= 0.0f ? max_dist * max_dist * 1.0001f : INFINITY);
        else
        for (int R = 2;; ++R) {
            bool touched;
            const unsigned long long lk = (R == 2) ? refine_shell<2>(tgt, cs_rsrc, pt_rsrc, 2, lg, x, y, z, cx, cy, cz, bestkey, touched)
                                                   : refine_shell<0>(tgt, cs_rsrc, pt_rsrc, R, lg, x, y, z, cx, cy, cz, bestkey, touched);
            bestkey = lk < bestkey ? lk : bestkey;
            const bool any_touched = (__ballot(touched) & gmask) != 0ull;
            const bool covers = (cx - R <= 0) && (cx + R >= g.gx - 1) && (cy - R <= 0) && (cy + R >= g.gy - 1) &&
                                (cz - R <= 0) && (cz + R >= g.gz - 1);
            const float big = 1.0e30f;
            const float mf = fmaxf(fminf(fminf(fminf(cx - R >= 1 ? fx : big, cx + R <= g.gx - 2 ? 1.0f - fx : big),
                                               fminf(cy - R >= 1 ? fy : big, cy + R <= g.gy - 2 ? 1.0f - fy : big)),
                                         fminf(cz - R >= 1 ? fz : big, cz + R <= g.gz - 2 ? 1.0f - fz : big)), 0.0f);
            const float bound = ((float)R + mf - 2e-3f) * g.h;
            const float bd = __uint_as_float((uint32_t)(bestkey >> 32));
#ifdef TC_REFINE_STATS
            if (lg == 0 && (covers || !any_touched || (bestkey != ~0ull && bd <= bound * bound + out2) || (max_dist >= 0.0f && bound > max_dist)))
                atomicAdd(const_cast<uint32_t *>(&st->refine_ring_hist[min(R, 7)]), 1u);
#endif
            if (covers || !any_touched) break;
            if (bestkey != ~0ull && bd <= bound * bound + out2) break;
            if (max_dist >= 0.0f && bound > max_dist) break;
            if (bestkey != ~0ull && !(dbg_shells)) {
                bestkey = refine_ball_scan(tgt, cs_rsrc, pt_rsrc, lg, x, y, z, bestkey, max_dist >= 0.0f ? max_dist * max_dist * 1.0001f : INFINITY);
                break;
            }
        }
        if (lg == 0) {
            const float best = __uint_as_float((uint32_t)(bestkey >> 32));
            const uint32_t bestg = (uint32_t)bestkey;
            bool valid = bestkey != ~0ull;
            if (valid && max_dist >= 0.0f) valid = !(sqrtf(best) > max_dist);
            corr_pos[4 * (size_t)j] = valid ? bestg : 0xFFFFFFFFu;
            if (valid) {
                const float4 c = tgt.pts[bestg];
                float a[NACC];
#pragma unroll
                for (int k = 0; k < NACC; ++k) a[k] = acc[k];
                if constexpr (MODE == 2) {
                    float R[9];
                    quat_to_rot(q, R);
                    accumulate_gicp(a, x, y, z, c, best, R, src_cov[2 * (size_t)j], src_cov[2 * (size_t)j + 1], tgt_nrm[2 * (size_t)bestg],
                                    tgt_nrm[2 * (size_t)bestg + 1]);
                } else {
                    float4 n = make_float4(0.f, 0.f, 0.f, 0.f);
                    if (P2PLANE) n = tgt_nrm[bestg];
                    accumulate_pair<P2PLANE, NACC>(g, a, x, y, z, c, n);
                }
#pragma unroll
                for (int k = 0; k < NACC; ++k) acc[k] = a[k];
            }
        }
    }
    __syncthreads();
    if (threadIdx.x < TC_ICP_SUMS_STRIDE) {
        double sum = 0.0;
        if (threadIdx.x < NACC) {
#pragma unroll 8
            for (int g2 = 0; g2 < kRefineThreads / kRG; ++g2) sum += (double)lacc[g2][threadIdx.x];
        }
        partial_rows[(size_t)blockIdx.x * TC_ICP_SUMS_STRIDE + threadIdx.x] = sum + folded;
    }
}

__global__ void __launch_bounds__(256) icp_write_corr_kernel(GridView tgt, const float4 *__restrict__ src, uint32_t ns,
                                                            const uint32_t *__restrict__ corr_pos,
                                                            uint32_t *__restrict__ corr) {
    const uint32_t j = blockIdx.x * blockDim.x + threadIdx.x;
    if (j >= ns) return;
    const uint32_t so = __float_as_uint(src[j].w);
    const uint32_t pj = corr_pos[4 * (size_t)j];
    corr[so] = (pj == 0xFFFFFFFFu) ? 0xFFFFFFFFu : __float_as_uint(tgt.pts[pj].w);
}

__global__ void __launch_bounds__(kIcpBlock) icp_final_mse_kernel(GridView tgt, const float4 *__restrict__ src, uint32_t ns,
                                                                  uint32_t chunk, const IcpState *__restrict__ st,
                                                                  const uint32_t *__restrict__ corr_pos,
                                                                  double *__restrict__ partials) {
    if (st->done) return;
    __shared__ double red[kIcpBlock / 64][TC_ICP_SUMS_STRIDE];
    const float q[4] = {st->q[0], st->q[1], st->q[2], st->q[3]};
    const float t[3] = {st->t[0], st->t[1], st->t[2]};
    double acc[2] = {0.0, 0.0};
    const uint32_t beg = blockIdx.x * chunk, end = min(beg + chunk, ns);
    for (uint32_t j = beg + threadIdx.x; j < end; j += kIcpBlock) {
        const float4 s = src[j];
        const uint32_t bj = __float_as_uint(s.w);
        if (bj == 0xFFFFFFFFu) continue;
        float x, y, z;
        isometry_apply(q, t, s.x, s.y, s.z, x, y, z);
        const float4 c = tgt.pts[bj];
        const float ex = x - c.x, ey = y - c.y, ez = z - c.z;
        acc[0] += (double)(ex * ex + ey * ey + ez * ez);
        acc[1] += 1.0;
    }
    block_reduce_store<2>(acc, partials + (size_t)blockIdx.x * TC_ICP_SUMS_STRIDE, red);
}

constexpr uint32_t kExactSumsMaxPairs = 4096;
constexpr uint32_t kExactSumsChunk = 4096;
constexpr int kExactSumsCols = TC_ICP_SUMS_P2P - 1;
static_assert(kRefineBlocks == kIcpBlock, "one lane per refine row reads the pair counts");
static inline uint32_t exact_sums_chunk(uint32_t ns) {
    const uint64_t per = ((uint64_t)ns + kRefineBlocks - 1) / kRefineBlocks;
    return (uint32_t)std::max<uint64_t>((per + kIcpBlock - 1) / kIcpBlock * kIcpBlock, kExactSumsChunk);
}
__global__ void __launch_bounds__(kIcpBlock) icp_exact_p2p_sums_kernel(GridView tgt, const float4 *__restrict__ src, uint32_t ns, uint32_t chunk,
                                                                       const IcpState *__restrict__ st, double *__restrict__ rows) {
    if (st->done) return;
    constexpr int NACC = kExactSumsCols;
    __shared__ double red[kIcpBlock / 64][TC_ICP_SUMS_STRIDE];
    __shared__ double wave_pairs[kIcpBlock / 64];
    const int lane = threadIdx.x & 63, w = threadIdx.x >> 6;
    {
        double v = rows[(size_t)threadIdx.x * TC_ICP_SUMS_STRIDE + (TC_ICP_SUMS_P2P - 1)];
#pragma unroll
        for (int o = 32; o > 0; o >>= 1) v += __shfl_xor(v, o);
        if (lane == 0) wave_pairs[w] = v;
    }
    __syncthreads();
    double pairs = 0.0;
#pragma unroll
    for (int w2 = 0; w2 < kIcpBlock / 64; ++w2) pairs += wave_pairs[w2];
    if (pairs > (double)kExactSumsMaxPairs) return;
    const float q[4] = {st->q[0], st->q[1], st->q[2], st->q[3]};
    const float t[3] = {st->t[0], st->t[1], st->t[2]};
    const double gc[3] = {(double)tgt.g.cx, (double)tgt.g.cy, (double)tgt.g.cz};
    double acc[NACC];
#pragma unroll
    for (int i = 0; i < NACC; ++i) acc[i] = 0.0;
    const uint64_t beg = (uint64_t)blockIdx.x * chunk, end = beg + chunk < (uint64_t)ns ? beg + chunk : (uint64_t)ns;
    for (uint64_t j = beg + threadIdx.x; j < end; j += kIcpBlock) {
        const float4 s = src[j];
        const uint32_t bj = __float_as_uint(s.w);
        if (bj == 0xFFFFFFFFu) continue;
        float x, y, z;
        isometry_apply(q, t, s.x, s.y, s.z, x, y, z);
        const float4 c = tgt.pts[bj];
        const double sv[3] = {(double)x - gc[0], (double)y - gc[1], (double)z - gc[2]};
        const double tv[3] = {(double)c.x - gc[0], (double)c.y - gc[1], (double)c.z - gc[2]};
#pragma unroll
        for (int r = 0; r < 3; ++r) {
            acc[r] += sv[r];
            acc[3 + r] += tv[r];
#pragma unroll
            for (int cc = 0; cc < 3; ++cc) acc[6 + 3 * r + cc] += sv[r] * tv[cc];
        }
        const float ex = x - c.x, ey = y - c.y, ez = z - c.z;
        acc[15] += (double)(ex * ex + ey * ey + ez * ez);
    }
#pragma unroll
    for (int i = 0; i < NACC; ++i) {
        double v = acc[i];
#pragma unroll
        for (int o = 32; o > 0; o >>= 1) v += __shfl_xor(v, o);
        acc[i] = v;
    }
    if (lane == 0) {
#pragma unroll
        for (int i = 0; i < NACC; ++i) red[w][i] = acc[i];
    }
    __syncthreads();
    if (threadIdx.x < NACC) {
        double sum = 0.0;
#pragma unroll
        for (int w2 = 0; w2 < kIcpBlock / 64; ++w2) sum += red[w2][threadIdx.x];
        rows[(size_t)blockIdx.x * TC_ICP_SUMS_STRIDE + threadIdx.x] = sum;
    }
    for (uint32_t r = gridDim.x + blockIdx.x; r < (uint32_t)kRefineBlocks; r += gridDim.x)
        if (threadIdx.x < NACC) rows[(size_t)r * TC_ICP_SUMS_STRIDE + threadIdx.x] = 0.0;
}

__global__ void __launch_bounds__(256) icp_target_nn_bound_kernel(GridView tgt, float4 *__restrict__ vor, const IcpState *__restrict__ st) {
    const uint32_t p = blockIdx.x * blockDim.x + threadIdx.x;
    const GridGeom &g = tgt.g;
    if (p >= g.n || (st && st->done)) return;
    const float4 q = tgt.pts[p];
    const int cx = cell_coord(q.x, g.minx, g.inv_h, g.gx), cy = cell_coord(q.y, g.miny, g.inv_h, g.gy), cz = cell_coord(q.z, g.minz, g.inv_h, g.gz);
    const int x0 = max(cx - 1, 0), x1 = min(cx + 1, g.gx - 1);
    const float hb = 0.996f * g.h;
    float m = hb * hb;
    for (int z = max(cz - 1, 0); z <= min(cz + 1, g.gz - 1); ++z)
        for (int y = max(cy - 1, 0); y <= min(cy + 1, g.gy - 1); ++y) {
            const uint32_t row = ((uint32_t)z * g.gy + y) * g.gx;
            const uint32_t s = tgt.cell_start[row + x0], e = tgt.cell_start[row + x1 + 1];
            for (uint32_t j = s; j < e; ++j) {
                const float4 c = tgt.pts[j];
                const float v = d2_nc(c.x, c.y, c.z, q.x, q.y, q.z);
                m = (j != p) ? fminf(m, v) : m;
            }
        }
    vor[p] = make_float4(q.x, q.y, q.z, 0.25f * 0.9999f * m);
}

__device__ __forceinline__ constexpr int tri(int r, int c) { return r * (r + 1) / 2 + c; }
__device__ __forceinline__ bool chol6_solve(const double *Su, const double *b, double (&x)[6]) {
    double L[21];
    {
        int o = 0;
#pragma unroll
        for (int r = 0; r < 6; ++r)
#pragma unroll
            for (int c = r; c < 6; ++c) { L[tri(c, r)] = Su[o]; ++o; }
    }
    bool ok = true;
    double rinv[6];
#pragma unroll
    for (int j = 0; j < 6; ++j) {
#pragma unroll
        for (int k = 0; k < j; ++k) {
            const double f = L[tri(j, k)];
#pragma unroll
            for (int r = j; r < 6; ++r) L[tri(r, j)] -= f * L[tri(r, k)];
        }
        const double d = L[tri(j, j)];
        ok = ok && (d > 0.0);
        const double dp = d > 0.0 ? d : 1.0;
        double inv = __builtin_amdgcn_rsq(dp);
        inv = inv * fma(-0.5 * dp * inv, inv, 1.5);
        inv = inv * fma(-0.5 * dp * inv, inv, 1.5);
        const double sd = dp * inv;
        rinv[j] = inv;
        L[tri(j, j)] = sd;
#pragma unroll
        for (int r = j + 1; r < 6; ++r) L[tri(r, j)] *= inv;
// ... 319 lines not shown

__global__ void icp_final_mse_fold_kernel(IcpState *__restrict__ st, const double *__restrict__ partials, uint32_t nblocks) {
    if (threadIdx.x >= TC_ICP_SUMS_STRIDE) return;
    double s = 0.0;
    if (threadIdx.x < 2 && !st->done)
        for (uint32_t b = 0; b < nblocks; ++b) s += partials[(size_t)b * TC_ICP_SUMS_STRIDE + threadIdx.x];
    st->sums[threadIdx.x] = s;
}

struct IcpLaunch {
    uint32_t nblocks = 0, chunk = 0;
    uint32_t mse_blocks = 0, mse_chunk = 0;
};
static IcpLaunch plan_launch(size_t ns) {
    IcpLaunch l;
    constexpr size_t kResidentBlocks = 4 * 256;
    size_t chunk = (ns + kResidentBlocks - 1) / kResidentBlocks;
    chunk = std::max<size_t>((chunk + kIcpBlock - 1) / kIcpBlock * kIcpBlock, kIcpBlock);
    uint32_t nb = (uint32_t)((ns + chunk - 1) / chunk);
    nb = std::max<uint32_t>((nb + 7) / 8 * 8, 8);
    l.nblocks = nb; l.chunk = (uint32_t)chunk;
    l.mse_blocks = nb; l.mse_chunk = (uint32_t)chunk;
    return l;
}

static TileGeom plan_tiles(const GridGeom &g, size_t ns) {
    const double rho = (double)ns / std::max<double>(g.ncell, 1.0);
    const double want = 256.0 / std::max(rho, 1e-6);
    static const int cand[][3] = {{8, 2, 2}, {8, 3, 2}, {8, 3, 3}, {8, 4, 3}, {8, 4, 4}, {8, 5, 4}, {8, 5, 5}, {8, 6, 5},
                                  {8, 6, 6}, {10, 6, 6}, {12, 6, 6}, {16, 6, 6}, {16, 8, 8}, {4, 2, 2}, {4, 2, 1}, {2, 2, 1}};
    int best = 0; double bd = 1e300;
    for (int i = 0; i < (int)(sizeof(cand) / sizeof(cand[0])); ++i) {
        const double c = (double)cand[i][0] * cand[i][1] * cand[i][2];
        const double d = std::fabs(std::log(c / want));
        if (d < bd) { bd = d; best = i; }
    }
    return make_tiles(g, cand[best][0], cand[best][1], cand[best][2]);
}

struct IcpSetup {
    int mode = 0;
    IcpLaunch l;
    GridView tv;
    TileGeom tg;
    DeviceIndex *tix = nullptr;
    const float4 *nrm = nullptr;
    const float4 *src = nullptr;
    float4 *wsrc = nullptr;
    uint32_t ns = 0;
    const float4 *src_cov = nullptr;
    float4 *wl = nullptr;
    IcpState *st = nullptr;
    uint32_t *rlist = nullptr;
    double *partials = nullptr;
};
static inline uint32_t *match_words(float4 *wsrc) { return reinterpret_cast<uint32_t *>(wsrc) + 3; }

enum class IcpStep { FullIteration, ReduceSum, ApplyOnly };

enum class MainVariant { Plain, Stats, Cert, Count };
static MainVariant main_variant(const IcpSetup &su, int dbg, bool want_cert, const int32_t *done_out) {
    if (dbg & 8) return MainVariant::Stats;
    const bool bounds = su.wl != nullptr && su.mode != 2;
    if (want_cert && bounds) return MainVariant::Cert;
    if (done_out != nullptr && bounds) return MainVariant::Count;
    return MainVariant::Plain;
}
using MainKernel = decltype(&icp_correspond_reduce_kernel<0>);
static MainKernel main_kernel(int mode, MainVariant v) {
    switch (v) {
    case MainVariant::Plain: return mode == 1 ? icp_correspond_reduce_kernel<1> : mode == 2 ? icp_correspond_reduce_kernel<2> : icp_correspond_reduce_kernel<0>;
    case MainVariant::Stats: return mode == 1 ? icp_correspond_reduce_kernel<1, true> : mode == 2 ? icp_correspond_reduce_kernel<2, true> : icp_correspond_reduce_kernel<0, true>;
    case MainVariant::Cert: return mode == 1 ? icp_correspond_reduce_kernel<1, false, true> : icp_correspond_reduce_kernel<0, false, true>;
    case MainVariant::Count: return mode == 1 ? icp_correspond_reduce_kernel<1, false, false, true> : icp_correspond_reduce_kernel<0, false, false, true>;
    }
    return nullptr;
}

static void launch_iteration(tc_context *ctx, const IcpSetup &su, IcpStep step, const float4 *vor = nullptr, int32_t *done_out = nullptr,
                             bool want_cert = false) {
    hipStream_t s = ctx->stream;
    const int dbg = debug_flags() | (ctx->profiling == 3 ? 8 : 0), mode = su.mode;
    const bool reduce_sum = step != IcpStep::ApplyOnly, apply = step != IcpStep::ReduceSum;
    const IcpLaunch &l = su.l;
    uint32_t *corr_pos = match_words(su.wsrc);
    double *refine_rows = su.partials + (size_t)l.nblocks * TC_ICP_SUMS_STRIDE;
    const MainVariant variant = main_variant(su, dbg, want_cert, done_out);
    if (reduce_sum) {
        {
            ProfScope ps(ctx, mode == 1 ? "icp_correspond_reduce_p2plane" : mode == 2 ? "icp_correspond_reduce_gicp" : "icp_correspond_reduce_p2p", true);
            const MainKernel kern = main_kernel(mode, variant);
            const float4 *vor_arg = (dbg & 4) ? nullptr : vor;
            unsigned long long *times_arg = (dbg & 1024) ? (unsigned long long *)ctx->dbg_times.p : nullptr;
            if (ps.active())
                hipExtLaunchKernelGGL(kern, dim3(l.nblocks), dim3(kIcpBlock), 0, s, ps.e0, ps.e1, 0, su.tv, su.nrm, su.wsrc, su.ns, l.chunk,
                                      (const IcpState *)su.st, su.rlist, su.partials, dbg, su.src_cov, vor_arg, times_arg, su.tv.pts12);
            else
                hipLaunchKernelGGL(kern, dim3(l.nblocks), dim3(kIcpBlock), 0, s, su.tv, su.nrm, su.wsrc, su.ns, l.chunk, su.st, su.rlist, su.partials, dbg,
                                   su.src_cov, vor_arg, times_arg, su.tv.pts12);
        }
        ProfScope ps(ctx, "icp_refine");
        auto kern = mode == 1 ? icp_refine_kernel<1> : mode == 2 ? icp_refine_kernel<2> : icp_refine_kernel<0>;
        hipLaunchKernelGGL(kern, dim3(kRefineBlocks), dim3(kRefineThreads), 0, s, su.tv, su.nrm, (const float4 *)su.wsrc, su.st, corr_pos, su.rlist, su.partials,
                           l.nblocks, l.chunk / (kIcpBlock / 64), refine_rows, su.src_cov, dbg);
        if (mode == 0 && !(dbg & 16)) {
            ProfScope ps2(ctx, "icp_exact_p2p_sums");
            const uint32_t chunk = exact_sums_chunk(su.ns);
            const uint32_t blocks = std::min<uint32_t>(std::max<uint32_t>((uint32_t)(((uint64_t)su.ns + chunk - 1) / chunk), 1u), (uint32_t)kRefineBlocks);
            hipLaunchKernelGGL(icp_exact_p2p_sums_kernel, dim3(blocks), dim3(kIcpBlock), 0, s, su.tv, (const float4 *)su.wsrc, su.ns, chunk,
                               (const IcpState *)su.st, refine_rows);
        }
    }
    ProfScope ps(ctx, "icp_finalize");
    const uint32_t rows = kRefineBlocks;
    auto kern = mode == 0 ? icp_finalize_kernel<0> : icp_finalize_kernel<1>;
    hipLaunchKernelGGL(kern, dim3(1), dim3(kFinalizeThreads), 0, s, refine_rows, rows, su.st, su.tv.g, reduce_sum ? 1 : 0, (apply && !(dbg & 32)) ? 1 : 0,
                       apply ? done_out : nullptr, (variant == MainVariant::Cert && reduce_sum) ? 1 : 0);
}

static size_t vor_after() {
    static const size_t v = [] { const char *e = getenv("TC_VOR_AFTER"); return e ? (size_t)atoi(e) : (size_t)6; }();
    return v;
}
static tc_status launch_target_nn_bounds(tc_context *ctx, DeviceIndex &ix, const GridView &tv, const IcpState *st, const float4 **out) {
    *out = nullptr;
    if (ix.vor_valid) { *out = (const float4 *)ix.vor.p; return TC_OK; }
    if (tc_status s = ensure(ctx, ix.vor, (size_t)ix.geom.n * sizeof(float4))) return s;
    ProfScope ps(ctx, "icp_target_nn_bounds");
    const bool persistent = &ix != &ctx->tgt_index;
    hipLaunchKernelGGL(icp_target_nn_bound_kernel, dim3((ix.geom.n + 255) / 256), dim3(256), 0, ctx->stream, tv, (float4 *)ix.vor.p,
                       persistent ? nullptr : st);
    ix.vor_valid = persistent;
    *out = (const float4 *)ix.vor.p;
    return TC_OK;
}

__global__ void __launch_bounds__(256) icp_pack12_kernel(const float4 *__restrict__ pts, uint32_t n, uint32_t npad, float *__restrict__ out) {
    const uint32_t i = blockIdx.x * blockDim.x + threadIdx.x;
    if (i >= npad) return;
    float4 r = make_float4(__uint_as_float(0x7F7F7F7Fu), __uint_as_float(0x7F7F7F7Fu), __uint_as_float(0x7F7F7F7Fu), 0.f);
    if (i < n) r = pts[i];
    out[3 * (size_t)i] = r.x; out[3 * (size_t)i + 1] = r.y; out[3 * (size_t)i + 2] = r.z;
}

__global__ void __launch_bounds__(256) icp_working_source_kernel(const float4 *__restrict__ src, uint32_t n, float4 *__restrict__ out, float4 *__restrict__ wl) {
    const uint32_t i = blockIdx.x * blockDim.x + threadIdx.x;
    if (i >= n) return;
    if (wl) wl[i] = make_float4(0.f, 0.f, 0.f, 0.f);
    float4 r = src[i];
    r.w = __uint_as_float(0xFFFFFFFFu);
    out[i] = r;
}

static tc_status icp_setup(tc_context *ctx, const IcpJob &job, const DeviceIndex *src_presorted, bool strict_source_order, IcpSetup &out) {
    const float *d_src = job.src, *d_tgt = job.tgt, *init = job.init;
    const size_t ns = job.ns, nt = job.nt;
    DeviceIndex *tgt_prebuilt = job.tgt_prebuilt;
    out.mode = job.mode;
    if (nt >= (1ull << 28) || ns >= (1ull << 28)) return fail(ctx, TC_UNSUPPORTED, "ICP clouds are limited to 2^28 - 1 points");
    out.tix = tgt_prebuilt ? tgt_prebuilt : &ctx->tgt_index;
    if (!tgt_prebuilt) {
        IndexSpec target_grid; target_grid.cell_factor = kIcpCellFactor; target_grid.target_ppo = 2.5f;
        if (tc_status s = build_index(ctx, ctx->tgt_index, d_tgt, nt, target_grid)) return s;
        if (tc_status s = wait_uploads(ctx)) return s;
        if (job.mode == 1)
            if (tc_status s = gather_normals(ctx, ctx->tgt_index, job.nrm, job.nstride)) return s;
    }
    if (tc_status s = wait_uploads(ctx)) return s;
    if (tc_status s = ensure(ctx, ctx->state, sizeof(IcpState))) return s;
    IcpState *hs = &pinned_host(ctx)->icp_staged;
    std::memset(hs, 0, sizeof(IcpState));
    for (int i = 0; i < 4; ++i) hs->q[i] = init[i];
    for (int i = 0; i < 3; ++i) hs->t[i] = init[4 + i];
    hs->prev_mse = INFINITY;
    hs->d_ang = -1.0f; hs->d_t = 0.0f; hs->d_run = 0;
    hs->conv_thr = job.conv_thr;
    hs->max_dist = job.max_dist;
    hs->kiss = job.kiss;
    hs->status = TC_OK;
    TC_HIP_TRY(ctx, hipMemcpyAsync(ctx->state.p, hs, sizeof(IcpState), hipMemcpyHostToDevice, ctx->stream));
    out.tg = plan_tiles((*out.tix).geom, ns);
    if (src_presorted && src_presorted->geom.n == ns) {
        out.src = (const float4 *)src_presorted->pts.p;
    } else {
        IndexSpec source_order;
        source_order.reuse_geom = &(*out.tix).geom; source_order.state_transform = (const IcpState *)ctx->state.p;
        source_order.tile_major = &out.tg; source_order.strict_order = strict_source_order;
        if (ns > 0)
            if (tc_status s = build_index(ctx, ctx->src_index, d_src, ns, source_order)) return s;
        out.src = (const float4 *)ctx->src_index.pts.p;
    }
    out.l = plan_launch(ns);
    if (tc_status s = ensure(ctx, ctx->partials, ((size_t)(kMaxPartialBlocks + kRefineBlocks) * TC_ICP_SUMS_STRIDE + 2) * sizeof(double))) return s;
    if (tc_status s = ensure(ctx, ctx->corr, (2 * ns + (size_t)kMaxPartialBlocks * (kIcpBlock / 64) + 4 + kRefineEntryWords * (size_t)out.l.nblocks * out.l.chunk) * sizeof(uint32_t))) return s;
    if (!out.tix->pts12_valid) {
        const uint32_t npad = (uint32_t)nt + 16u;
        if (tc_status s = ensure(ctx, out.tix->pts12, (size_t)npad * 12 + 64)) return s;
        ProfScope ps(ctx, "icp_pack12");
        hipLaunchKernelGGL(icp_pack12_kernel, dim3((npad + 255) / 256), dim3(256), 0, ctx->stream, (const float4 *)(*out.tix).pts.p, (uint32_t)nt, npad,
                           (float *)out.tix->pts12.p);
        out.tix->pts12_valid = true;
    }
    out.tv = view_of((*out.tix));
    if (tc_status s = ensure(ctx, ctx->icp_wsrc, 2 * (ns + 4) * sizeof(float4))) return s;
    out.wsrc = (float4 *)ctx->icp_wsrc.p;
    if (ns > 0) {
        ProfScope ps(ctx, "icp_working_source");
        hipLaunchKernelGGL(icp_working_source_kernel, dim3((unsigned)((ns + 255) / 256)), dim3(256), 0, ctx->stream, out.src, (uint32_t)ns, out.wsrc, (float4 *)nullptr);
    }
    out.ns = (uint32_t)ns;
    out.nrm = (const float4 *)out.tix->normals.p;
    out.st = (IcpState *)ctx->state.p;
    out.rlist = (uint32_t *)ctx->corr.p + 2 * ns;
    out.partials = (double *)ctx->partials.p;
    return TC_OK;
}

__global__ void __launch_bounds__(256) gather_cov_kernel(const float4 *__restrict__ pts_sorted, uint32_t n, const float4 *__restrict__ cov_orig,
                                                        float4 *__restrict__ out) {
    const uint32_t i = blockIdx.x * blockDim.x + threadIdx.x;
    if (i >= n) return;
    const uint32_t o = __float_as_uint(pts_sorted[i].w);
    out[2 * (size_t)i] = cov_orig[2 * (size_t)o];
    out[2 * (size_t)i + 1] = cov_orig[2 * (size_t)o + 1];
}

static void fold_search_stats(tc_context *ctx, const IcpState *hs) {
    if (!((debug_flags() & 8) || ctx->profiling == 3)) return;
    const uint32_t *h = hs->refine_ring_hist;
    unsigned long long needed;
    std::memcpy(&needed, &h[3], sizeof(needed));
    ctx->stat_icp[0] += hs->iterations; ctx->stat_icp[1] += h[5]; ctx->stat_icp[2] += h[6]; ctx->stat_icp[3] += h[7];
    ctx->stat_icp[4] += needed; ctx->stat_icp[5] += h[2];
    if (debug_flags() & 8)
        fprintf(stderr, "[tc] icp main pass over %u iterations: wave trips %u, without a search %u (%.1f %%); searches %u, candidate steps needed %llu "
                        "(%.2f per search), steps taken by the trips' slowest lanes %u (%.2f per searching trip): lock-step ratio (lane slots spent / steps needed) %.2f\n",
                hs->iterations, h[5], h[6], 100.0 * h[6] / std::max(h[5], 1u), h[7], needed, (double)needed / std::max(h[7], 1u), h[2],
                (double)h[2] / std::max(h[5] - h[6], 1u), (double)h[2] * 64.0 / std::max<double>((double)needed, 1.0));
}

static tc_status launch_finish(tc_context *ctx, const IcpSetup &su, uint32_t mse_blocks, int from_sums, bool via_staged_copy, const IcpState **out) {
    PinnedBlock *pb = pinned_host(ctx);
    IcpState *hs = via_staged_copy ? &pb->icp_staged : &pb->icp_result, *hs_dev = nullptr;
    if (!via_staged_copy) {
        hs_dev = (IcpState *)pinned_dev_ptr(ctx, hs);
        if (!hs_dev) return fail(ctx, TC_GPU, "ICP: the pinned block has no device address");
        hs->status = TC_GPU; hs->iterations = 0;
    }
    const bool direct = !via_staged_copy && pinned_poll_enabled();
    hipLaunchKernelGGL(icp_finish_kernel, dim3(1), dim3(64), 0, ctx->stream, su.st, (const double *)su.partials, mse_blocks, su.mode != 0 ? 1 : 0, from_sums,
                       direct ? hs_dev : (IcpState *)nullptr);
    if (!direct) TC_HIP_TRY(ctx, hipMemcpyAsync(hs, su.st, sizeof(IcpState), hipMemcpyDeviceToHost, ctx->stream));
    *out = hs;
    return TC_OK;
}

static tc_status fill_result(tc_context *ctx, const IcpState *hs, size_t max_iters, const char *failed, bool check_count, tc_icp_result *res) {
    if (hs->status != TC_OK) return fail(ctx, (tc_status)hs->status, failed);
    if (check_count && !hs->converged && hs->iterations != max_iters)
        return fail(ctx, TC_GPU, "internal error: the ICP loop executed " + std::to_string(hs->iterations) + " of " + std::to_string(max_iters) + " iterations");
    for (int i = 0; i < 4; ++i) res->transformation[i] = hs->q[i];
    for (int i = 0; i < 3; ++i) res->transformation[4 + i] = hs->t[i];
    res->mse = hs->mse;
    res->iterations = hs->converged ? hs->iterations : max_iters;
    res->converged = hs->converged;
    res->n_correspondences = hs->n_corr;
    return TC_OK;
}

template <typename F>
static tc_status run_chunked(tc_context *ctx, size_t max_iters, F &&enqueue_iteration) {
    auto chunk_len = [](size_t c) -> size_t { return c == 0 ? 6 : c == 1 ? 2 : c <= 4 ? 4 : 8; };
    size_t nchunks = 0;
    for (size_t covered = 0; covered < max_iters; ++nchunks) covered += chunk_len(nchunks);
    volatile int32_t *flags = pinned_host(ctx)->icp_flags;
    int32_t *d_flags = nullptr;
    TC_HIP_TRY(ctx, hipHostGetDevicePointer((void **)&d_flags, (void *)flags, 0));
    const size_t max_flags = kIcpMaxFlags;
    size_t it = 0;
    const bool sticky = ctx->icp_cert_hint && nchunks >= 3;
    ctx->icp_cert = sticky;
    struct Hint { tc_context *c; bool wanted; ~Hint() { c->icp_cert_hint = wanted; } } hint{ctx, sticky};
    for (size_t c = 0; c < nchunks; ++c) {
        if (c >= 2 && c - 2 < max_flags) {
            if (tc_status s = wait_pinned_word(ctx, (volatile uint32_t *)&flags[c - 2], "ICP loop")) return s;
            if (flags[c - 2] == 1) break;
            hint.wanted = flags[c - 2] == 3;
            ctx->icp_cert = sticky || hint.wanted;
        }
        if (c < max_flags) flags[c] = 0;
        for (size_t k = 0; k < chunk_len(c) && it < max_iters; ++k, ++it) {
            const bool last = k + 1 == chunk_len(c) || it + 1 == max_iters;
            if (tc_status s = enqueue_iteration((last && c < max_flags) ? d_flags + c : nullptr)) return s;
        }
    }
    return TC_OK;
}

static void dump_block_schedule(tc_context *ctx, uint32_t nblocks) {
    std::vector<unsigned long long> h(2 * (size_t)nblocks);
    (void)hipMemcpy(h.data(), ctx->dbg_times.p, h.size() * sizeof(unsigned long long), hipMemcpyDeviceToHost);
    unsigned long long t0 = ~0ull, t1 = 0;
    for (size_t b = 0; b < nblocks; ++b) { t0 = std::min(t0, h[2 * b]); t1 = std::max(t1, h[2 * b + 1]); }
    std::vector<double> dur, endt, startt;
    for (size_t b = 0; b < nblocks; ++b) { dur.push_back((h[2 * b + 1] - h[2 * b]) * 0.01); endt.push_back((h[2 * b + 1] - t0) * 0.01); startt.push_back((h[2 * b] - t0) * 0.01); }
    std::sort(dur.begin(), dur.end()); std::sort(endt.begin(), endt.end()); std::sort(startt.begin(), startt.end());
    auto q = [](const std::vector<double> &v, double f) { return v[(size_t)(f * (v.size() - 1))]; };
    fprintf(stderr, "[tc] main pass blocks: %u; span %.1f us; block duration us min %.1f p10 %.1f p50 %.1f p90 %.1f p99 %.1f max %.1f; start p50 %.1f p99 %.1f max %.1f; end p10 %.1f p50 %.1f p90 %.1f\n",
            nblocks, (t1 - t0) * 0.01, dur.front(), q(dur, 0.1), q(dur, 0.5), q(dur, 0.9), q(dur, 0.99), dur.back(), q(startt, 0.5), q(startt, 0.99), startt.back(),
            q(endt, 0.1), q(endt, 0.5), q(endt, 0.9));
#ifdef TC_PHASE_STAMPS
    {
        std::vector<unsigned long long> hp(8 * (size_t)nblocks);
        (void)hipMemcpy(hp.data(), (unsigned long long *)ctx->dbg_times.p + 2 * kMaxPartialBlocks, hp.size() * sizeof(unsigned long long), hipMemcpyDeviceToHost);
        double m[8] = {0};
        for (size_t b = 0; b < nblocks; ++b) for (int i = 0; i < 8; ++i) m[i] += (double)hp[8 * b + i] / nblocks;
        fprintf(stderr, "[tc]   wave 0 phases, mean s_memtime ticks: stage1-2 %.0f  windows %.0f  loop %.0f  post %.0f  stage4 %.0f  fold %.0f  end %.0f\n", m[0], m[1], m[2], m[3], m[4], m[5], m[6]);
    }
#endif
    fprintf(stderr, "[tc]   per XCD (block & 7): mean duration / last end, us:");
    for (int x = 0; x < 8; ++x) {
        double sum = 0, last = 0; int cnt = 0;
        for (size_t b = x; b < nblocks; b += 8) { sum += (h[2 * b + 1] - h[2 * b]) * 0.01; last = std::max(last, (h[2 * b + 1] - t0) * 0.01); ++cnt; }
        fprintf(stderr, " %.1f/%.1f", sum / std::max(cnt, 1), last);
    }
    fprintf(stderr, "\n");
}

tc_status icp_run(tc_context *ctx, const IcpJob &job, tc_icp_result *res) {
    const int mode = job.mode;
    const size_t ns = job.ns, nt = job.nt;
    IcpSetup su;
    if (tc_status s = icp_setup(ctx, job, mode == 2 ? nullptr : job.src_presorted, false, su)) return s;
    su.wl = su.wsrc + ns + 4;
    hipStream_t st = ctx->stream;
    uint32_t *corr = (uint32_t *)ctx->corr.p, *corr_pos = match_words(su.wsrc);
    if (mode == 2) {
        if (tc_status s = ensure(ctx, (*su.tix).normals, nt * 2 * sizeof(float4))) return s;
        if (tc_status s = ensure(ctx, ctx->gicp_src_cov, ns * 2 * sizeof(float4))) return s;
        hipLaunchKernelGGL(gather_cov_kernel, dim3((unsigned)((nt + 255) / 256)), dim3(256), 0, st, (const float4 *)(*su.tix).pts.p,
                           (uint32_t)nt, (const float4 *)job.cov_tgt, (float4 *)(*su.tix).normals.p);
        hipLaunchKernelGGL(gather_cov_kernel, dim3((unsigned)((ns + 255) / 256)), dim3(256), 0, st, su.src, (uint32_t)ns,
                           (const float4 *)job.cov_src, (float4 *)ctx->gicp_src_cov.p);
        su.src_cov = (const float4 *)ctx->gicp_src_cov.p;
        su.nrm = (const float4 *)(*su.tix).normals.p;
    }

    size_t enq = 0;
    const float4 *vor = su.tix->vor_valid ? (const float4 *)su.tix->vor.p : nullptr;
    if (debug_flags() & 1024)
        if (tc_status s = ensure(ctx, ctx->dbg_times, 10 * (size_t)kMaxPartialBlocks * sizeof(unsigned long long))) return s;
    if (tc_status s = run_chunked(ctx, job.max_iters, [&](int32_t *done_out) -> tc_status {
            if (enq++ == vor_after() && !vor)
                if (tc_status s = launch_target_nn_bounds(ctx, (*su.tix), su.tv, su.st, &vor)) return s;
            launch_iteration(ctx, su, IcpStep::FullIteration, vor, done_out, ctx->icp_cert);
            return TC_OK;
        })) return s;
    if (mode == 0) {
        ProfScope ps(ctx, "icp_final_mse");
        hipLaunchKernelGGL(icp_final_mse_kernel, dim3(su.l.mse_blocks), dim3(kIcpBlock), 0, st, su.tv, (const float4 *)su.wsrc, (uint32_t)ns,
                           su.l.mse_chunk, su.st, corr_pos, su.partials);
    }
    const IcpState *hs = nullptr;
    if (tc_status s = launch_finish(ctx, su, su.l.mse_blocks, 0, false, &hs)) return s;
    if (res->corr_target) {
        hipLaunchKernelGGL(icp_write_corr_kernel, dim3((unsigned)((ns + 255) / 256)), dim3(256), 0, st, su.tv, su.src, (uint32_t)ns,
                           corr_pos, job.corr_on_device ? res->corr_target : corr);
        if (!job.corr_on_device) TC_HIP_TRY(ctx, hipMemcpyAsync(res->corr_target, corr, ns * sizeof(uint32_t), hipMemcpyDeviceToHost, st));
    }
    TC_HIP_TRY(ctx, hipStreamSynchronize(st));
    TC_HIP_TRY(ctx, hipGetLastError());
    if ((debug_flags() & 1024) && ctx->dbg_times.p) dump_block_schedule(ctx, su.l.nblocks);
    fold_search_stats(ctx, hs);
    if (debug_flags() & 64)
        fprintf(stderr, "[tc] icp: searching lanes at the last evaluation of the certificate's gate %u (d_run %u, wanted %d)\n", hs->searchers, hs->d_run, hs->d_ang >= 0.0f ? 1 : 0);
    if (debug_flags() & 64)
        fprintf(stderr, "[tc] icp: %u iterations, refine queries total %u max %u  exit ring hist %u %u %u %u %u %u %u %u\n", hs->iterations,
                hs->refine_total, hs->refine_max, hs->refine_ring_hist[0], hs->refine_ring_hist[1], hs->refine_ring_hist[2], hs->refine_ring_hist[3],
                hs->refine_ring_hist[4], hs->refine_ring_hist[5], hs->refine_ring_hist[6], hs->refine_ring_hist[7]);
    return fill_result(ctx, hs, job.max_iters,
                       mode == 2 ? "GICP: insufficient correspondences (need >= 6) or ill-conditioned Gauss-Newton system"
                       : mode == 1 ? "Insufficient correspondences for point-to-plane ICP (need >= 6) or ill-conditioned system"
                                   : "Insufficient correspondences found", true, res);
}


__global__ void __launch_bounds__(256) icp_zero_u32_kernel(uint32_t *__restrict__ p, uint32_t n) {
    const uint32_t i = blockIdx.x * blockDim.x + threadIdx.x;
    if (i < n) p[i] = 0u;
}

tc_status icp_run_sharded(tc_context *ctx, tc_comm *comm, int shard_mode, const IcpJob &job, tc_icp_result *res) {
    const int mode = job.mode;
    const size_t ns = job.ns, max_iters = job.max_iters;
    const int W = comm ? comm->nranks : 1, rank = comm ? comm->rank : 0;
    IcpSetup su;
    const size_t rows = (ns + (size_t)W - 1) / (size_t)W;
    size_t ilo = 0, ihi = ns;
    if (shard_mode == TC_SHARD_INDEX) { ilo = std::min((size_t)rank * rows, ns); ihi = std::min(ilo + rows, ns); }
    const size_t n_setup = ihi - ilo;
    IcpJob mine = job;
    mine.src = job.src + 3 * ilo; mine.ns = n_setup;
    tc_status setup_rc = icp_setup(ctx, mine, nullptr, shard_mode == TC_SHARD_SPATIAL && W > 1, su);
    if (setup_rc == TC_OK && !su.tix->vor_valid) setup_rc = ensure(ctx, su.tix->vor, (size_t)su.tix->geom.n * sizeof(float4));
    const bool gather_index = shard_mode == TC_SHARD_INDEX && res->corr_target && ns > 0 && (W > 1 || (comm && comm->nccl));
    if (setup_rc == TC_OK && gather_index) setup_rc = ensure(ctx, ctx->out_a, (size_t)W * rows * sizeof(uint32_t));
    if (tc_status s = comm_agree(comm, setup_rc)) return s;
    hipStream_t st = ctx->stream;
    size_t lo = 0, hi = n_setup;
    if (shard_mode == TC_SHARD_SPATIAL) { lo = ns * (size_t)rank / (size_t)W; hi = ns * ((size_t)rank + 1) / (size_t)W; }
    const size_t nl = hi - lo;
    su.src += lo; su.wsrc += lo; su.ns = (uint32_t)nl; su.l = plan_launch(nl);
    const IcpLaunch &l = su.l;
    uint32_t *corr = (uint32_t *)ctx->corr.p, *corr_pos = match_words(su.wsrc);
    size_t enq = 0;
    const float4 *vor = su.tix->vor_valid ? (const float4 *)su.tix->vor.p : nullptr;
    if (tc_status s = run_chunked(ctx, max_iters, [&](int32_t *done_out) -> tc_status {
            if (enq++ == vor_after() && !vor)
                if (tc_status s = launch_target_nn_bounds(ctx, (*su.tix), su.tv, su.st, &vor)) return s;
            launch_iteration(ctx, su, IcpStep::ReduceSum, vor);
            if (tc_status s = comm_allreduce_f64(comm, su.st->sums, TC_ICP_SUMS_STRIDE)) return s;
            launch_iteration(ctx, su, IcpStep::ApplyOnly, nullptr, done_out);
            return TC_OK;
        })) return s;
    if (mode == 0) {
        hipLaunchKernelGGL(icp_final_mse_kernel, dim3(l.mse_blocks), dim3(kIcpBlock), 0, st, su.tv, (const float4 *)su.wsrc, (uint32_t)nl, l.mse_chunk, su.st,
                           corr_pos, su.partials);
        hipLaunchKernelGGL(icp_final_mse_fold_kernel, dim3(1), dim3(64), 0, st, su.st, su.partials, l.mse_blocks);
        if (tc_status s = comm_allreduce_f64(comm, su.st->sums, TC_ICP_SUMS_STRIDE)) return s;
    }
    const IcpState *hs = nullptr;
    if (tc_status s = launch_finish(ctx, su, 0u, 1, false, &hs)) return s;
    if (res->corr_target && ns > 0) {
        if (gather_index) {
            uint32_t *all = (uint32_t *)ctx->out_a.p;
            if (nl > 0)
                hipLaunchKernelGGL(icp_write_corr_kernel, dim3((unsigned)((nl + 255) / 256)), dim3(256), 0, st, su.tv, su.src, (uint32_t)nl, corr_pos,
                                   all + (size_t)rank * rows);
            if (tc_status s = comm_allgather(comm, all, rows * sizeof(uint32_t))) return s;
            TC_HIP_TRY(ctx, hipMemcpyAsync(res->corr_target, all, ns * sizeof(uint32_t), hipMemcpyDeviceToDevice, st));
        } else {
            const bool gather = shard_mode == TC_SHARD_SPATIAL && (W > 1 || (comm && comm->nccl));
            if (gather) hipLaunchKernelGGL(icp_zero_u32_kernel, dim3((unsigned)((ns + 255) / 256)), dim3(256), 0, st, corr, (uint32_t)ns);
            if (nl > 0)
                hipLaunchKernelGGL(icp_write_corr_kernel, dim3((unsigned)((nl + 255) / 256)), dim3(256), 0, st, su.tv, su.src, (uint32_t)nl, corr_pos, corr);
            if (gather)
                if (tc_status s = comm_allreduce_u32(comm, corr, ns)) return s;
            TC_HIP_TRY(ctx, hipMemcpyAsync(res->corr_target, corr, n_setup * sizeof(uint32_t), hipMemcpyDeviceToDevice, st));
        }
    }
    TC_HIP_TRY(ctx, hipStreamSynchronize(st));
    TC_HIP_TRY(ctx, hipGetLastError());
    fold_search_stats(ctx, hs);
    return fill_result(ctx, hs, max_iters, mode == 1 ? "Insufficient correspondences for point-to-plane ICP (need >= 6) or ill-conditioned system"
                                                     : "Insufficient correspondences found", true, res);
}

}

struct tc_icp_shard {
    tc_context *ctx;
    tc::IcpSetup su;
};

extern "C" {

tc_status tc_icp_shard_create(tc_context *ctx, int point_to_plane, const float *d_source_slice, size_t n_source_slice,
                              const float *d_target, size_t n_target, const float *d_target_normals, size_t normal_stride,
                              const float init[7], float max_correspondence_distance, float convergence_threshold,
                              tc_icp_shard **out) try {
    if (!ctx || !out) return TC_INVALID_DATA;
    if (n_source_slice == 0 || n_target == 0) return tc::fail(ctx, TC_INVALID_DATA, "Source or target point cloud is empty");
    if (!point_to_plane) return tc::fail(ctx, TC_UNSUPPORTED, "tc_icp_shard_*: point-to-plane only; use tc_sharded_icp_detailed_device");
    tc::IcpJob job;
    job.mode = 1;
    job.src = d_source_slice; job.ns = n_source_slice;
    job.tgt = d_target; job.nt = n_target;
    job.nrm = d_target_normals; job.nstride = normal_stride;
    job.init = init; job.max_dist = max_correspondence_distance; job.conv_thr = convergence_threshold;
    tc_icp_shard *s = new tc_icp_shard{ctx, {}};
    tc_status rc = tc::icp_setup(ctx, job, nullptr, false, s->su);
    if (rc != TC_OK) { delete s; return rc; }
    *out = s;
    return TC_OK;
} TC_CATCH_STATUS(ctx)

double *tc_icp_shard_sums(tc_icp_shard *s) { return ((tc::IcpState *)s->ctx->state.p)->sums; }

tc_status tc_icp_shard_get_sums(tc_icp_shard *s, double *d_out) try {
    tc_context *ctx = s->ctx;
    TC_HIP_TRY(ctx, hipMemcpyAsync(d_out, ((tc::IcpState *)ctx->state.p)->sums, TC_ICP_SUMS_STRIDE * sizeof(double),
                                   hipMemcpyDeviceToDevice, ctx->stream));
    return TC_OK;
} TC_CATCH_STATUS((s ? s->ctx : nullptr))

tc_status tc_icp_shard_set_sums(tc_icp_shard *s, const double *d_in) try {
    tc_context *ctx = s->ctx;
    TC_HIP_TRY(ctx, hipMemcpyAsync(((tc::IcpState *)ctx->state.p)->sums, d_in, TC_ICP_SUMS_STRIDE * sizeof(double),
                                   hipMemcpyDeviceToDevice, ctx->stream));
    return TC_OK;
} TC_CATCH_STATUS((s ? s->ctx : nullptr))

tc_status tc_icp_shard_done(tc_icp_shard *s, int *done) try {
    tc_context *ctx = s->ctx;
    if (tc_status rc = tc::read_back(ctx, &tc::pinned_host(ctx)->count, &((tc::IcpState *)ctx->state.p)->done, sizeof(int32_t))) return rc;
    *done = (int32_t)tc::pinned_host(ctx)->count;
    return TC_OK;
} TC_CATCH_STATUS((s ? s->ctx : nullptr))

tc_status tc_icp_shard_reduce(tc_icp_shard *s) try {
    tc_context *ctx = s->ctx;
    tc::launch_iteration(ctx, s->su, tc::IcpStep::ReduceSum);
    TC_HIP_TRY(ctx, hipGetLastError());
    return TC_OK;
} TC_CATCH_STATUS((s ? s->ctx : nullptr))

tc_status tc_icp_shard_apply(tc_icp_shard *s) try {
    tc_context *ctx = s->ctx;
    tc::launch_iteration(ctx, s->su, tc::IcpStep::ApplyOnly);
    TC_HIP_TRY(ctx, hipGetLastError());
    return TC_OK;
} TC_CATCH_STATUS((s ? s->ctx : nullptr))

tc_status tc_icp_shard_finish(tc_icp_shard *s, size_t max_iters, tc_icp_result *res) try {
    tc_context *ctx = s->ctx;
    hipStream_t st = ctx->stream;
    const tc::IcpSetup &su = s->su;
    const tc::IcpState *hs = nullptr;
    if (tc_status rc = tc::launch_finish(ctx, su, 0u, 0, true, &hs)) return rc;
    if (res->corr_target) {
        uint32_t *corr = (uint32_t *)ctx->corr.p;
        hipLaunchKernelGGL(tc::icp_write_corr_kernel, dim3((unsigned)((su.ns + 255) / 256)), dim3(256), 0, st, su.tv, su.src, su.ns,
                           tc::match_words(su.wsrc), corr);
        TC_HIP_TRY(ctx, hipMemcpyAsync(res->corr_target, corr, su.ns * sizeof(uint32_t), hipMemcpyDeviceToDevice, st));
    }
    TC_HIP_TRY(ctx, hipStreamSynchronize(st));
    tc::fold_search_stats(ctx, hs);
    return tc::fill_result(ctx, hs, max_iters, "ICP failed (insufficient correspondences / singular system)", false, res);
} TC_CATCH_STATUS((s ? s->ctx : nullptr))

void tc_icp_shard_destroy(tc_icp_shard *s) { delete s; }

}
```

threecrate_amd/csrc/tc_internal.h:

```cpp
#pragma once
#include <hip/hip_runtime.h>
#include <stddef.h>
#include <stdint.h>
#include <new>
#include <exception>
#include <string>
#include <type_traits>
#include <vector>

#include "../../include/threecrate_hip.h"

namespace tc {

struct GridGeom {
    float minx, miny, minz;
    float maxx, maxy, maxz;
    float h, inv_h;
    int   gx, gy, gz;
    uint32_t ncell;
    uint32_t n;
    float cx, cy, cz;
    int   clamped;
};

// ... 121 lines not shown
    uint32_t n_long;
    uint32_t alive;
    uint32_t taken;
    uint32_t n_out_vertices;
    uint32_t pad[11];
};
static_assert(sizeof(QemOut) == 64, "");

struct AlphaOut {
    uint32_t flags;
    uint32_t boundary;
    uint64_t pairs;
    uint64_t candidates;
    uint32_t faces;
    uint32_t pad[9];
};
static_assert(sizeof(AlphaOut) == 64, "");

constexpr size_t kIcpMaxFlags = 200;
struct PinnedBlock {
    char     reserved[256];
    IcpState icp_staged;
    IcpState icp_result;
    union {
        volatile int32_t icp_flags[kIcpMaxFlags];
        uint32_t count;
        uint32_t filter_out[2];
        PlaneOut plane_out;
    };
    char     pad_flags[1024 - kIcpMaxFlags * sizeof(int32_t)];
    float    bbox[30];
    char     pad_bbox[8192 - 30 * sizeof(float)];
    volatile uint32_t occ[2];
    char     pad_occ[56];
    uint32_t big_cell;
    char     pad_big[60];
    uint32_t agree;
    char     pad_agree[60];
    volatile uint32_t bbox_done;
    char     pad_done[60];
    volatile uint32_t bin_max[2];
    char     pad_bin[56];
    NdtBuildOut ndt_build;
    NdtState ndt_state;
    TsdfOut  tsdf_out;
    RansacOut ransac_out;
    VoxelMapOut voxelmap_out;
    ColorOut color_out;
    MeshOut  mesh_out;
    SimplifyOut simplify_out;
    McOut    mc_out;
    QemOut   qem_out;
    AlphaOut alpha_out;
};
constexpr size_t kPinnedBytes = 1 << 16;
static_assert(offsetof(PinnedBlock, icp_staged) == 256 && offsetof(PinnedBlock, icp_result) == 640 && offsetof(PinnedBlock, icp_flags) == 1024 &&
              offsetof(PinnedBlock, count) == 1024 && offsetof(PinnedBlock, filter_out) == 1024 && offsetof(PinnedBlock, plane_out) == 1024 &&
              sizeof(PlaneOut) <= sizeof(PinnedBlock::icp_flags) && offsetof(PinnedBlock, bbox) == 2048 && offsetof(PinnedBlock, occ) == 2048 + 8192 &&
              offsetof(PinnedBlock, big_cell) == 2048 + 8192 + 64 && offsetof(PinnedBlock, agree) == 2048 + 8192 + 128 &&
              offsetof(PinnedBlock, bbox_done) == 2048 + 8192 + 192 && offsetof(PinnedBlock, bin_max) == 2048 + 8192 + 256 &&
              offsetof(PinnedBlock, ndt_build) == 2048 + 8192 + 320 && offsetof(PinnedBlock, ndt_state) == 2048 + 8192 + 384 &&
              offsetof(PinnedBlock, tsdf_out) == 2048 + 8192 + 480 && offsetof(PinnedBlock, ransac_out) == 2048 + 8192 + 544 &&
              offsetof(PinnedBlock, voxelmap_out) == 2048 + 8192 + 608 && offsetof(PinnedBlock, color_out) == 2048 + 8192 + 672 &&
              offsetof(PinnedBlock, mesh_out) == 2048 + 8192 + 736 && offsetof(PinnedBlock, simplify_out) == 2048 + 8192 + 800 &&
              offsetof(PinnedBlock, mc_out) == 2048 + 8192 + 864 && offsetof(PinnedBlock, qem_out) == 2048 + 8192 + 928 &&
              offsetof(PinnedBlock, alpha_out) == 2048 + 8192 + 992,
              "a region of the pinned block has moved");
static_assert(offsetof(PinnedBlock, icp_result) - offsetof(PinnedBlock, icp_staged) >= sizeof(IcpState) &&
              offsetof(PinnedBlock, icp_flags) - offsetof(PinnedBlock, icp_result) >= sizeof(IcpState),
              "an IcpState slot of the pinned block is too small: the staged state would run into the result, the result into the chunk flags");
static_assert(sizeof(PinnedBlock::icp_flags) == kIcpMaxFlags * sizeof(int32_t) &&
              offsetof(PinnedBlock, icp_flags) + sizeof(PinnedBlock::icp_flags) <= offsetof(PinnedBlock, bbox), "the chunk flags run into the bounding box");
static_assert(sizeof(PinnedBlock) <= kPinnedBytes, "the pinned block outgrew its allocation");
constexpr int kIcpBlock = 256;
constexpr int kTsdfBlock = 256, kTsdfRun = 64;
constexpr size_t kTsdfMaxVoxels = (size_t)1 << 28;
constexpr size_t kPtsPad = 4, kCellStartPad = 4;
constexpr size_t kCellStartFront = 4;
constexpr uint32_t kRankQuadraticMax = 1u << 20;
constexpr int kMaxPartialBlocks = 1024;
constexpr uint32_t kAdaptMinPoints = 1u << 18;

#if defined(__HIPCC__)
__device__ __forceinline__ uint32_t tile_major_id(const TileGeom &t, int cx, int cy, int cz) {
    const int ax = cx / t.tx, ay = cy / t.ty, az = cz / t.tz;
    const int lx = cx - ax * t.tx, ly = cy - ay * t.ty, lz = cz - az * t.tz;
    const uint32_t tile = ((uint32_t)az * t.nty + ay) * t.ntx + ax;
    return tile * t.cpt + ((uint32_t)lz * t.ty + ly) * t.tx + lx;
}
__device__ __forceinline__ float d2_nc(float ax, float ay, float az, float bx, float by, float bz) {
    float dx = ax - bx, dy = ay - by, dz = az - bz;
    return dx * dx + dy * dy + dz * dz;
}
__device__ __forceinline__ int cell_coord(float v, float mn, float inv_h, int g) {
    float f = (v - mn) * inv_h;
    int c = (f >= 0.0f) ? (int)f : 0;
    return c < g ? c : g - 1;
}
__device__ __forceinline__ void isometry_apply(const float q[4], const float t[3], float x, float y, float z,
                                               float &ox, float &oy, float &oz) {
    float tx = (q[1] * z - q[2] * y) * 2.0f;
    float ty = (q[2] * x - q[0] * z) * 2.0f;
    float tz = (q[0] * y - q[1] * x) * 2.0f;
    float cx = q[1] * tz - q[2] * ty;
    float cy = q[2] * tx - q[0] * tz;
    float cz = q[0] * ty - q[1] * tx;
    ox = ((tx * q[3] + cx) + x) + t[0];
    oy = ((ty * q[3] + cy) + y) + t[1];
    oz = ((tz * q[3] + cz) + z) + t[2];
}
__device__ __forceinline__ void store_compacted(const float *__restrict__ xyz, uint32_t i, uint32_t o, float *__restrict__ out_xyz,
                                                uint32_t *__restrict__ out_index) {
    if (out_xyz) {
        out_xyz[3 * (size_t)o] = xyz[3 * (size_t)i]; out_xyz[3 * (size_t)o + 1] = xyz[3 * (size_t)i + 1]; out_xyz[3 * (size_t)o + 2] = xyz[3 * (size_t)i + 2];
    }
    if (out_index) out_index[o] = i;
}
typedef float f32x3 __attribute__((ext_vector_type(3)));
__device__ __forceinline__ __amdgpu_buffer_rsrc_t raw_rsrc(const void *p) {
    return __builtin_amdgcn_make_buffer_rsrc(const_cast<void *>(p), 0, 0xFFFFFFFF, 0x00020000);
}
#endif

struct DevBuf {
    void  *p = nullptr;
    size_t cap = 0;
};

struct ScopedBuf : DevBuf {
    ScopedBuf() = default;
    ScopedBuf(const ScopedBuf &) = delete; ScopedBuf &operator=(const ScopedBuf &) = delete;
    ~ScopedBuf() { if (p) (void)hipFree(p); }
};

struct KernelTimer {
    std::string name;
    std::vector<std::pair<hipEvent_t, hipEvent_t>> pending;
    uint64_t launches = 0;
    double   total_ms = 0.0;
    double   min_ms = 1e300, max_ms = 0.0;
};

struct DeviceIndex {
    GridGeom geom{};
    TileGeom tile{};
    float exact_min[3] = {0, 0, 0}, exact_max[3] = {0, 0, 0};
    DevBuf pts;
    DevBuf cell_start;
    DevBuf normals;
    DevBuf vor;
    bool vor_valid = false;
    DevBuf pts12;
    bool pts12_valid = false;
    uint32_t occ_host = 0;
    bool occ_host_valid = false;
    DevBuf cell_of;
    DevBuf slot;
    DevBuf arrival;
    DevBuf fill;
    DevBuf blocksum;
};
struct IndexSpec {
    float cell_factor = 0.0f;
    float min_cell_edge = 0.0f;
    float target_ppo = 0.0f;
    const GridGeom *reuse_geom = nullptr;
    const IcpState *state_transform = nullptr;
    const TileGeom *tile_major = nullptr;
    bool strict_order = false;
};
__host__ __device__ inline int ball_rings(const GridGeom &g, float radius) {
    const int gyz = g.gy > g.gz ? g.gy : g.gz;
    return (int)fminf(ceilf(radius * g.inv_h) + 1.0f, (float)(g.gx > gyz ? g.gx : gyz));
}
template <class F> void for_each_scratch_buf(DeviceIndex &ix, F f) { for (DevBuf *b : {&ix.cell_of, &ix.slot, &ix.arrival, &ix.fill, &ix.blocksum}) f(*b); }
template <class F> void for_each_buf(DeviceIndex &ix, F f) {
    for (DevBuf *b : {&ix.pts, &ix.cell_start, &ix.normals, &ix.vor, &ix.pts12}) f(*b);
    for_each_scratch_buf(ix, f);
}

enum CluSlot {
    CLU_PARENT, CLU_SIZE, CLU_MIN_INDEX,
    CLU_FLAG, CLU_POS,
    CLU_KEYS,
    CLU_ROOTS,
    CLU_RANK_OF, CLU_SIZES,
    CLU_LABELS, CLU_SORT_TEMP, CLU_COMP,
    CLU_SLOTS
};
enum FpfhSlot {
    FPFH_XYZ, FPFH_SPFH, FPFH_MODE,
    FPFH_FB_POS, FPFH_FB_XYZ, FPFH_FB_COUNT,
    FPFH_SORTED_OF,
    FPFH_KNN_IDX, FPFH_KNN_DIST, FPFH_KNN_COUNT,
    FPFH_SLOTS
};

enum VoxSlot {
    VOX_KEYS,
    VOX_KEYS_SORTED,
    VOX_INDEX,
    VOX_ORDER,
    VOX_FLAG,
    VOX_POS,
    VOX_START,
    VOX_SORT_TEMP,
    VOX_BLOCKSUM,
    VOX_SLOTS
};

}

struct tc_context {
    int device = 0;
    hipStream_t stream = nullptr;
    bool own_stream = true;
    std::string last_error;
    int profiling = 0;
    uint32_t prof_tick = 0;
    std::vector<tc::KernelTimer> timers;
    std::vector<hipEvent_t> event_pool;
    std::vector<tc::DevBuf> pool;
    size_t pool_bytes = 0;
    size_t pool_largest = 0;
    hipEvent_t order_event = nullptr;
    hipEvent_t release_event = nullptr;
    std::vector<hipEvent_t> chunk_events;
    hipStream_t copy_stream = nullptr;
    hipEvent_t upload_event = nullptr;
    bool upload_pending = false;
    bool upload_used_copy_stream = false;

    tc::DeviceIndex tgt_index;
    tc::DeviceIndex src_index;
    tc::DevBuf in_a, in_b, in_c;
    tc::DevBuf out_a;
    tc::DevBuf bbox;
    tc::DevBuf state;
    tc::DevBuf partials;
    tc::DevBuf corr;
    tc::DevBuf gicp_src_cov;
    tc::DevBuf icp_wsrc;
    tc::DevBuf dbg_times;
    tc::DevBuf overflow;
    tc::DevBuf build_tmp;
    tc::DevBuf normals_hard;
    unsigned long long stat_indexed_points = 0, stat_index_builds = 0;
    unsigned long long stat_icp[6] = {0, 0, 0, 0, 0, 0};
    bool icp_cert = false;
    bool icp_cert_hint = false;
    bool normals_hard_clean = false;
    tc::DevBuf vox[tc::VOX_SLOTS];
    tc::DevBuf clu[tc::CLU_SLOTS];
    tc::DevBuf fpfh[tc::FPFH_SLOTS];
    tc::DevBuf fpfh_np;
    void *pinned = nullptr;
    void *pinned_dev = nullptr;
};
template <class F> void for_each_buf(tc_context &c, F f) {
    for (tc::DeviceIndex *ix : {&c.tgt_index, &c.src_index}) tc::for_each_buf(*ix, f);
    for (auto &b : c.vox) f(b);
    for (auto &b : c.clu) f(b);
    for (auto &b : c.fpfh) f(b);
    for (tc::DevBuf *b : {&c.fpfh_np, &c.in_a, &c.in_b, &c.in_c, &c.out_a, &c.bbox, &c.state, &c.partials, &c.corr, &c.gicp_src_cov,
                          &c.overflow, &c.normals_hard, &c.build_tmp, &c.dbg_times, &c.icp_wsrc}) f(*b);
}

struct tc_comm {
    tc_context *ctx = nullptr;
    int rank = 0, nranks = 1;
    void *nccl = nullptr;
    bool own_nccl = false;
    tc_host_collective_fn host_fn = nullptr;
    void *host_user = nullptr;
    void *agree_word = nullptr;
};

namespace tc {

tc_status fail(tc_context *ctx, tc_status st, const std::string &msg);
tc_status fail_nothrow(tc_context *ctx, tc_status st, const char *msg) noexcept;
void fault_point(const char *site);
#define TC_CATCH_STATUS(CTX)                                                                                            \
    catch (const std::bad_alloc &) { return tc::fail_nothrow((CTX), TC_GPU, "out of host memory"); }                    \
    catch (const std::exception &e_) { return tc::fail_nothrow((CTX), TC_GPU, e_.what()); }                             \
    catch (...) { return tc::fail_nothrow((CTX), TC_GPU, "unknown C++ exception"); }
#define TC_CATCH_VOID catch (...) { }
#define TC_CATCH_VALUE(V) catch (...) { return V; }
#define TC_HIP_TRY(ctx, expr)                                                                  \
    do {                                                                                       \
        hipError_t _e = (expr);                                                                \
        if (_e != hipSuccess)                                                                  \
            return tc::fail((ctx), TC_GPU, std::string(#expr) + ": " + hipGetErrorString(_e)); \
    } while (0)

tc_status ensure(tc_context *ctx, DevBuf &b, size_t bytes);
constexpr size_t kMaxPoints = 0xFFFFFFF0ull, kMaxK = 2048;
inline tc_status check_point_count(tc_context *ctx, size_t a, size_t b = 0) {
    return (a >= kMaxPoints || b >= kMaxPoints) ? fail(ctx, TC_UNSUPPORTED, "more than 2^32 points") : TC_OK;
}
tc_status upload_async(tc_context *ctx, void *d_dst, const void *h_src, size_t bytes);
tc_status uploads_issued(tc_context *ctx);
tc_status wait_uploads(tc_context *ctx);
inline PinnedBlock *pinned_host(tc_context *ctx) { return static_cast<PinnedBlock *>(ctx->pinned); }
void *pinned_dev_ptr(tc_context *ctx, const void *host_addr);
bool pinned_poll_enabled();
tc_status wait_pinned_word(tc_context *ctx, volatile uint32_t *word, const char *what);
tc_status read_back(tc_context *ctx, void *host_dst, const void *dev_src, size_t bytes);
tc_status stage_in(tc_context *ctx, DevBuf &b, const void *h_src, size_t bytes);
tc_status synced(tc_context *ctx);
tc_status stage_out(tc_context *ctx, void *h_dst, const void *d_src, size_t bytes);
void recycle(tc_context *ctx, DevBuf &b);

struct ProfScope {
    tc_context *ctx; int idx = -1; hipEvent_t e0 = nullptr, e1 = nullptr; bool ext = false;
    ProfScope(tc_context *c, const char *name, bool dominant = false);
    ~ProfScope();
    bool active() const { return idx >= 0; }
};

tc_status build_index(tc_context *ctx, DeviceIndex &ix, const float *d_xyz, size_t n, const IndexSpec &spec);
TileGeom make_tiles(const GridGeom &g, int tx, int ty, int tz);
tc_status gather_normals(tc_context *ctx, DeviceIndex &ix, const float *d_normals, size_t stride);
GridView view_of(const DeviceIndex &ix);
template <class F> void with_clamped(const GridView &gv, F launch) {
    if (gv.g.clamped) launch(std::true_type{});
    else launch(std::false_type{});
}

tc_status exclusive_scan_u32(tc_context *ctx, const uint32_t *d_in, uint32_t n, uint32_t *d_out , DevBuf &blocksum, uint32_t *occ_out = nullptr,
// ... 84 lines not shown
```

Before: 18090 it/s.

## Fuse packed-xyz, original-index and working-source writes into index build placement

The index build's placement kernels now also write a packed 12-byte xyz copy and an original-index array for ICP targets. For the source index they also write the ICP working-source copy, so the separate pts12 and icp_working_source passes are skipped. The initial ICP state is seeded from kernel arguments inside the first build kernel rather than by a host-to-device memcpy. Correspondence writing reads original indices from the compact array instead of the float4 points. This removes extra full-array passes and a small H2D copy, at the cost of more stores in the placement kernels and added coupling between build and ICP setup.

```diff
diff --git a/threecrate_amd/csrc/api.hip b/threecrate_amd/csrc/api.hip
--- a/threecrate_amd/csrc/api.hip
+++ b/threecrate_amd/csrc/api.hip
@@ -243,7 +243,7 @@
 
 void recycle_index(tc_context *ctx, DeviceIndex &ix) {
     for_each_buf(ix, [ctx](DevBuf &b) { recycle(ctx, b); });
-    ix.pts12_valid = false; ix.vor_valid = false;
+    ix.pts12_valid = false; ix.orig_valid = false; ix.vor_valid = false;
 }
 
 void free_index(DeviceIndex &ix) { for_each_buf(ix, free_buf); }
diff --git a/threecrate_amd/csrc/cloud.hip b/threecrate_amd/csrc/cloud.hip
--- a/threecrate_amd/csrc/cloud.hip
+++ b/threecrate_amd/csrc/cloud.hip
@@ -50,6 +50,7 @@
     }
     c->has_normals = false;
     IndexSpec spec; spec.cell_factor = f; spec.min_cell_edge = min_h; spec.target_ppo = target_ppo;
+    spec.icp_target = true;
     if (tc_status s = build_index(ctx, c->ix, (const float *)c->xyz.p, c->n, spec)) return s;
     c->indexed = true;
     c->factor = f;
diff --git a/threecrate_amd/csrc/grid.hip b/threecrate_amd/csrc/grid.hip
--- a/threecrate_amd/csrc/grid.hip
+++ b/threecrate_amd/csrc/grid.hip
@@ -114,11 +114,43 @@
 }
 
 
+constexpr uint32_t kPts12Pad = 16;
+struct __attribute__((packed, aligned(4))) Packed12 { float x, y, z; };
+__device__ __forceinline__ void store_place_extras(const PlaceExtras &ex, uint32_t pos, float4 r) {
+    if (ex.pts12) *reinterpret_cast<Packed12 *>(ex.pts12 + 3 * (size_t)pos) = Packed12{r.x, r.y, r.z};
+    if (ex.orig) ex.orig[pos] = __float_as_uint(r.w);
+    if (ex.wsrc) { r.w = __uint_as_float(0xFFFFFFFFu); ex.wsrc[pos] = r; }
+}
+__device__ __forceinline__ void store_seed_state(const IcpSeed &seed, IcpState *st) {
+    for (uint32_t w = threadIdx.x; w < sizeof(IcpState) / sizeof(uint32_t); w += blockDim.x) {
+        uint32_t v = 0u;
+        switch (w) {
+        case 0: v = __float_as_uint(seed.q[0]); break;
+        case 1: v = __float_as_uint(seed.q[1]); break;
+        case 2: v = __float_as_uint(seed.q[2]); break;
+        case 3: v = __float_as_uint(seed.q[3]); break;
+        case 4: v = __float_as_uint(seed.t[0]); break;
+        case 5: v = __float_as_uint(seed.t[1]); break;
+        case 6: v = __float_as_uint(seed.t[2]); break;
+        case offsetof(IcpState, prev_mse) / 4: v = 0x7F800000u; break;
+        case offsetof(IcpState, conv_thr) / 4: v = __float_as_uint(seed.conv_thr); break;
+        case offsetof(IcpState, max_dist) / 4: v = __float_as_uint(seed.max_dist); break;
+        case offsetof(IcpState, kiss) / 4: v = (uint32_t)seed.kiss; break;
+        case offsetof(IcpState, d_ang) / 4: v = 0xBF800000u; break;
+        default: break;
+        }
+        reinterpret_cast<uint32_t *>(st)[w] = v;
+    }
+}
+static_assert(offsetof(IcpState, q) == 0 && offsetof(IcpState, t) == 16 && sizeof(IcpState) % sizeof(uint32_t) == 0 && TC_OK == 0,
+              "store_seed_state writes the pose by word number and the status as a zero word");
+
 __global__ void __launch_bounds__(256) cell_hist_kernel(const float *__restrict__ xyz, uint32_t n, GridGeom g,
                                                        const IcpState *__restrict__ st, TileGeom tg, int tile_major, uint32_t nkeys,
                                                        uint32_t *__restrict__ cell_of, uint32_t *__restrict__ hist,
                                                        uint32_t *__restrict__ arrival, uint32_t *__restrict__ pts_pad,
-                                                       uint32_t *__restrict__ cs_front, uint32_t *__restrict__ cs_tail, uint32_t rank_max) {
+                                                       uint32_t *__restrict__ cs_front, uint32_t *__restrict__ cs_tail, uint32_t rank_max,
+                                                       uint32_t *__restrict__ pts12_pad, IcpSeed seed) {
     uint32_t i = blockIdx.x * blockDim.x + threadIdx.x;
     if (blockIdx.x == 0 && threadIdx.x < 4 * kPtsPad + kCellStartFront + kCellStartPad) {
         const uint32_t t = threadIdx.x;
@@ -126,10 +158,14 @@
         else if (t < 4 * kPtsPad + kCellStartFront) cs_front[t - 4 * kPtsPad] = 0u;
         else cs_tail[t - 4 * kPtsPad - kCellStartFront] = 0u;
     }
+    if (blockIdx.x == 0 && pts12_pad && threadIdx.x < 3 * kPts12Pad) pts12_pad[threadIdx.x] = 0x7F7F7F7Fu;
+    if (blockIdx.x == 0 && seed.store) store_seed_state(seed, const_cast<IcpState *>(st));
     if (i >= n) return;
     float x = xyz[3 * (size_t)i], y = xyz[3 * (size_t)i + 1], z = xyz[3 * (size_t)i + 2];
     if (st) {
-        float q[4] = {st->q[0], st->q[1], st->q[2], st->q[3]}, t[3] = {st->t[0], st->t[1], st->t[2]};
+        float q[4], t[3];
+        if (seed.store) { q[0] = seed.q[0]; q[1] = seed.q[1]; q[2] = seed.q[2]; q[3] = seed.q[3]; t[0] = seed.t[0]; t[1] = seed.t[1]; t[2] = seed.t[2]; }
+        else { q[0] = st->q[0]; q[1] = st->q[1]; q[2] = st->q[2]; q[3] = st->q[3]; t[0] = st->t[0]; t[1] = st->t[1]; t[2] = st->t[2]; }
         float ox, oy, oz;
         isometry_apply(q, t, x, y, z, ox, oy, oz);
         x = ox; y = oy; z = oz;
@@ -252,7 +288,7 @@
                                                          const uint32_t *__restrict__ cell_of,
                                                          const uint32_t *__restrict__ cell_start,
                                                          const uint32_t *__restrict__ slot,
-                                                         float4 *__restrict__ pts, int slot_is_ordered, uint32_t rank_max) {
+                                                         float4 *__restrict__ pts, int slot_is_ordered, uint32_t rank_max, PlaceExtras ex) {
     uint32_t p = blockIdx.x * blockDim.x + threadIdx.x;
     if (p >= n) return;
     uint32_t i = slot[p];
@@ -272,6 +308,7 @@
     if (c == nkeys) r.x = r.y = r.z = __uint_as_float(0x7F7F7F7Fu);
     r.w = __uint_as_float(i);
     pts[s + rank] = r;
+    store_place_extras(ex, s + rank, r);
 }
 
 __global__ void __launch_bounds__(256) place_kernel(const float *__restrict__ xyz, uint32_t n, uint32_t nkeys,
@@ -290,7 +327,7 @@
 
 __global__ void __launch_bounds__(256) rerank_kernel(uint32_t n, GridGeom g, const IcpState *__restrict__ st, TileGeom tg, int tile_major,
                                                     uint32_t nkeys, const uint32_t *__restrict__ cell_start, const float4 *__restrict__ tmp,
-                                                    float4 *__restrict__ pts, uint32_t rank_max) {
+                                                    float4 *__restrict__ pts, uint32_t rank_max, PlaceExtras ex) {
     const uint32_t p = blockIdx.x * blockDim.x + threadIdx.x;
     if (p >= n) return;
     const float4 r = tmp[p];
@@ -318,6 +355,7 @@
         rank = p - s;
     }
     pts[s + rank] = r;
+    store_place_extras(ex, s + rank, r);
 }
 
 __global__ void __launch_bounds__(256) gather_normals_kernel(const float4 *__restrict__ pts, uint32_t n,
@@ -567,11 +605,24 @@
     if (!(fabsf(x) <= 3.0e38f && fabsf(y) <= 3.0e38f && fabsf(z) <= 3.0e38f)) c = nkeys;
     return c;
 }
+__device__ __forceinline__ uint32_t point_key_at(float x, float y, float z, const GridGeom &g, const float *q, const float *t, const TileGeom &tg,
+                                                 int tile_major, uint32_t nkeys) {
+    if (q) {
+        float ox, oy, oz;
+        isometry_apply(q, t, x, y, z, ox, oy, oz);
+        x = ox; y = oy; z = oz;
+    }
+    const int ix = cell_coord(x, g.minx, g.inv_h, g.gx), iy = cell_coord(y, g.miny, g.inv_h, g.gy), iz = cell_coord(z, g.minz, g.inv_h, g.gz);
+    uint32_t c = tile_major ? tile_major_id(tg, ix, iy, iz) : ((uint32_t)iz * g.gy + iy) * g.gx + ix;
+    if (!(fabsf(x) <= 3.0e38f && fabsf(y) <= 3.0e38f && fabsf(z) <= 3.0e38f)) c = nkeys;
+    return c;
+}
 
 __global__ void __launch_bounds__(kBinWalkThreads) bin_count_kernel(const float *__restrict__ xyz, uint32_t n, GridGeom g, const IcpState *__restrict__ st,
                                                        TileGeom tg, int tile_major, uint32_t nkeys, uint32_t kpb, uint32_t nbins,
                                                        uint32_t *__restrict__ cnt , uint32_t *__restrict__ pts_pad,
-                                                       uint32_t *__restrict__ cs_front, uint32_t *__restrict__ cs_tail) {
+                                                       uint32_t *__restrict__ cs_front, uint32_t *__restrict__ cs_tail,
+                                                       uint32_t *__restrict__ pts12_pad, IcpSeed seed) {
     __shared__ uint32_t c[kBinMaxBins];
     if (blockIdx.x == 0 && threadIdx.x < 4 * kPtsPad + kCellStartFront + kCellStartPad) {
         const uint32_t t = threadIdx.x;
@@ -579,12 +630,17 @@
         else if (t < 4 * kPtsPad + kCellStartFront) cs_front[t - 4 * kPtsPad] = 0u;
         else cs_tail[t - 4 * kPtsPad - kCellStartFront] = 0u;
     }
+    if (blockIdx.x == 0 && pts12_pad && threadIdx.x < 3 * kPts12Pad) pts12_pad[threadIdx.x] = 0x7F7F7F7Fu;
+    if (blockIdx.x == 0 && seed.store) store_seed_state(seed, const_cast<IcpState *>(st));
+    float q[4] = {0.f, 0.f, 0.f, 1.f}, t[3] = {0.f, 0.f, 0.f};
+    if (seed.store) { q[0] = seed.q[0]; q[1] = seed.q[1]; q[2] = seed.q[2]; q[3] = seed.q[3]; t[0] = seed.t[0]; t[1] = seed.t[1]; t[2] = seed.t[2]; }
+    else if (st) { q[0] = st->q[0]; q[1] = st->q[1]; q[2] = st->q[2]; q[3] = st->q[3]; t[0] = st->t[0]; t[1] = st->t[1]; t[2] = st->t[2]; }
     for (uint32_t b = threadIdx.x; b < nbins; b += kBinWalkThreads) c[b] = 0u;
     __syncthreads();
     const uint32_t per = (n + kBinBlocks - 1) / kBinBlocks;
     const uint32_t i0 = blockIdx.x * per, i1 = min(i0 + per, n);
     for (uint32_t i = i0 + threadIdx.x; i < i1; i += kBinWalkThreads) {
-        const uint32_t k = point_key(xyz[3 * (size_t)i], xyz[3 * (size_t)i + 1], xyz[3 * (size_t)i + 2], g, st, tg, tile_major, nkeys);
+        const uint32_t k = point_key_at(xyz[3 * (size_t)i], xyz[3 * (size_t)i + 1], xyz[3 * (size_t)i + 2], g, st ? q : nullptr, t, tg, tile_major, nkeys);
         atomicAdd(&c[min(k / kpb, nbins - 1u)], 1u);
     }
     __syncthreads();
@@ -673,7 +729,7 @@
                                                                      const IcpState *__restrict__ st, TileGeom tg, int tile_major,
                                                                      uint32_t *__restrict__ cs, float4 *__restrict__ pts,
                                                                      uint32_t *__restrict__ occ_ticket, uint32_t *__restrict__ occ_out,
-                                                                     unsigned long long *__restrict__ occ_host) {
+                                                                     unsigned long long *__restrict__ occ_host, PlaceExtras ex) {
     __shared__ uint32_t cnt[kBinKeysMax];
     __shared__ uint32_t rkey[kBinCap];
     __shared__ uint32_t ridx[kBinCap];
@@ -737,7 +793,11 @@
     __syncthreads();
     for (uint32_t i = tid; i < P; i += kBinPlaceThreads) slot[rkey[i]] = i;
     __syncthreads();
-    for (uint32_t t = tid; t < P; t += kBinPlaceThreads) pts[bs + t] = tmp[bs + slot[t]];
+    for (uint32_t t = tid; t < P; t += kBinPlaceThreads) {
+        const float4 r = tmp[bs + slot[t]];
+        pts[bs + t] = r;
+        store_place_extras(ex, bs + t, r);
+    }
     if (tid == 0) {
         const unsigned long long mine = ((unsigned long long)s_occ << 32) | 1ull;
         const unsigned long long old = __hip_atomic_fetch_add(reinterpret_cast<unsigned long long *>(occ_ticket), mine, __ATOMIC_RELAXED, __HIP_MEMORY_SCOPE_AGENT);
@@ -765,12 +825,29 @@
     ctx->stat_index_builds += 1;
     ix.vor_valid = false;
     ix.pts12_valid = false;
+    ix.orig_valid = false;
     ix.occ_host_valid = false;
     hipStream_t st = ctx->stream;
     const uint32_t n32 = (uint32_t)n;
     const int nb = (int)((n + 255) / 256);
     const int dbg = debug_flags();
     const uint32_t rank_max = rank_quadratic_max();
+    PlaceExtras ex{nullptr, nullptr, spec.working_copy};
+    uint32_t *pts12_pad = nullptr;
+    if (spec.icp_target) {
+        if (tc_status s = ensure(ctx, ix.pts12, (n + kPts12Pad) * 12 + 64)) return s;
+        if (tc_status s = ensure(ctx, ix.orig, n * sizeof(uint32_t))) return s;
+        ex.pts12 = (float *)ix.pts12.p; ex.orig = (uint32_t *)ix.orig.p;
+        pts12_pad = reinterpret_cast<uint32_t *>(ex.pts12 + 3 * n);
+    }
+    IcpSeed seed{};
+    if (spec.state_init && spec.state_transform) {
+        const IcpState &h = *spec.state_init;
+        for (int i = 0; i < 4; ++i) seed.q[i] = h.q[i];
+        for (int i = 0; i < 3; ++i) seed.t[i] = h.t[i];
+        seed.conv_thr = h.conv_thr; seed.max_dist = h.max_dist; seed.kiss = h.kiss; seed.store = 1;
+    }
+    const IcpSeed no_seed{};
 
     if (spec.reuse_geom) {
         ix.geom = *spec.reuse_geom;
@@ -834,7 +911,8 @@
                 {
                     ProfScope ps(ctx, "cell_bin_count");
                     hipLaunchKernelGGL(bin_count_kernel, dim3(kBinBlocks), dim3(kBinWalkThreads), 0, st, d_xyz, n32, g, spec.state_transform, tg, spec.tile_major ? 1 : 0, nkeys, kpb,
-                                       nbins, cnt, reinterpret_cast<uint32_t *>((float4 *)ix.pts.p + n), (uint32_t *)ix.cell_start.p, cs + nkeys + 2);
+                                       nbins, cnt, reinterpret_cast<uint32_t *>((float4 *)ix.pts.p + n), (uint32_t *)ix.cell_start.p, cs + nkeys + 2, pts12_pad, seed);
+                    seed = no_seed;
                 }
                 {
                     ProfScope ps(ctx, "cell_bin_offsets");
@@ -852,7 +930,7 @@
                     ProfScope ps(ctx, "cell_bin_place");
                     hipLaunchKernelGGL(bin_place_kernel, dim3(nbins), dim3(kBinPlaceThreads), 0, st, (const float4 *)ctx->build_tmp.p, (const uint32_t *)binstart,
                                        nbins, kpb, nkeys, g, spec.state_transform, tg, spec.tile_major ? 1 : 0, cs, (float4 *)ix.pts.p, occ_ticket,
-                                       (uint32_t *)ix.cell_start.p, d_occ_host);
+                                       (uint32_t *)ix.cell_start.p, d_occ_host, ex);
                 }
                 TC_HIP_TRY(ctx, hipGetLastError());
                 if (tc_status s = wait_pinned_word(ctx, h_max + 1, "index build (bin populations)")) return s;
@@ -869,7 +947,8 @@
             ProfScope ps(ctx, "cell_hist");
             hipLaunchKernelGGL(cell_hist_kernel, dim3(nb), dim3(256), 0, st, d_xyz, n32, g, spec.state_transform, tg, spec.tile_major ? 1 : 0, nkeys,
                                (uint32_t *)ix.cell_of.p, (uint32_t *)ix.fill.p, (uint32_t *)ix.arrival.p,
-                               reinterpret_cast<uint32_t *>((float4 *)ix.pts.p + n), (uint32_t *)ix.cell_start.p, cs + nkeys + 2, rank_max);
+                               reinterpret_cast<uint32_t *>((float4 *)ix.pts.p + n), (uint32_t *)ix.cell_start.p, cs + nkeys + 2, rank_max, pts12_pad, seed);
+            seed = no_seed;
         }
         {
             ProfScope ps(ctx, "cell_scan");
@@ -887,7 +966,7 @@
         {
             ProfScope ps(ctx, "cell_rerank");
             hipLaunchKernelGGL(rerank_kernel, dim3(nb), dim3(256), 0, st, n32, g, spec.state_transform, tg, spec.tile_major ? 1 : 0, nkeys, (const uint32_t *)cs,
-                               (const float4 *)ctx->build_tmp.p, (float4 *)ix.pts.p, rank_max);
+                               (const float4 *)ctx->build_tmp.p, (float4 *)ix.pts.p, rank_max, ex);
         }
         }
         TC_HIP_TRY(ctx, hipGetLastError());
@@ -924,10 +1003,11 @@
                                          bits_for_value(nkeys_final), ix.blocksum)) return s;
             ProfScope ps(ctx, "cell_rank_gather_strict");
             hipLaunchKernelGGL(rank_gather_kernel, dim3(nb), dim3(256), 0, st, d_xyz, n32, nkeys_final, (const uint32_t *)ix.cell_of.p,
-                               (const uint32_t *)cs_final, (const uint32_t *)ix.slot.p, (float4 *)ix.pts.p, 1, rank_max);
+                               (const uint32_t *)cs_final, (const uint32_t *)ix.slot.p, (float4 *)ix.pts.p, 1, rank_max, ex);
             TC_HIP_TRY(ctx, hipGetLastError());
         }
     }
+    ix.pts12_valid = ix.orig_valid = spec.icp_target;
     return TC_OK;
 }
 
diff --git a/threecrate_amd/csrc/icp.hip b/threecrate_amd/csrc/icp.hip
--- a/threecrate_amd/csrc/icp.hip
+++ b/threecrate_amd/csrc/icp.hip
@@ -1001,12 +1001,12 @@
 
 __global__ void __launch_bounds__(256) icp_write_corr_kernel(GridView tgt, const float4 *__restrict__ src, uint32_t ns,
                                                             const uint32_t *__restrict__ corr_pos,
-                                                            uint32_t *__restrict__ corr) {
+                                                            uint32_t *__restrict__ corr, const uint32_t *__restrict__ orig) {
     const uint32_t j = blockIdx.x * blockDim.x + threadIdx.x;
     if (j >= ns) return;
     const uint32_t so = __float_as_uint(src[j].w);
     const uint32_t pj = corr_pos[4 * (size_t)j];
-    corr[so] = (pj == 0xFFFFFFFFu) ? 0xFFFFFFFFu : __float_as_uint(tgt.pts[pj].w);
+    corr[so] = (pj == 0xFFFFFFFFu) ? 0xFFFFFFFFu : orig ? orig[pj] : __float_as_uint(tgt.pts[pj].w);
 }
 
 __global__ void __launch_bounds__(kIcpBlock) icp_final_mse_kernel(GridView tgt, const float4 *__restrict__ src, uint32_t ns,
@@ -1632,7 +1632,7 @@
     out[i] = r;
 }
 
-static tc_status icp_setup(tc_context *ctx, const IcpJob &job, const DeviceIndex *src_presorted, bool strict_source_order, IcpSetup &out) {
+static tc_status icp_setup(tc_context *ctx, const IcpJob &job, const DeviceIndex *src_presorted, bool strict_source_order, bool fused, IcpSetup &out) {
     const float *d_src = job.src, *d_tgt = job.tgt, *init = job.init;
     const size_t ns = job.ns, nt = job.nt;
     DeviceIndex *tgt_prebuilt = job.tgt_prebuilt;
@@ -1640,7 +1640,7 @@
     if (nt >= (1ull << 28) || ns >= (1ull << 28)) return fail(ctx, TC_UNSUPPORTED, "ICP clouds are limited to 2^28 - 1 points");
     out.tix = tgt_prebuilt ? tgt_prebuilt : &ctx->tgt_index;
     if (!tgt_prebuilt) {
-        IndexSpec target_grid; target_grid.cell_factor = kIcpCellFactor; target_grid.target_ppo = 2.5f;
+        IndexSpec target_grid; target_grid.cell_factor = kIcpCellFactor; target_grid.target_ppo = 2.5f; target_grid.icp_target = fused;
         if (tc_status s = build_index(ctx, ctx->tgt_index, d_tgt, nt, target_grid)) return s;
         if (tc_status s = wait_uploads(ctx)) return s;
         if (job.mode == 1)
@@ -1658,7 +1658,10 @@
     hs->max_dist = job.max_dist;
     hs->kiss = job.kiss;
     hs->status = TC_OK;
-    TC_HIP_TRY(ctx, hipMemcpyAsync(ctx->state.p, hs, sizeof(IcpState), hipMemcpyHostToDevice, ctx->stream));
+    const bool build_source = !(src_presorted && src_presorted->geom.n == ns) && ns > 0;
+    const bool seed_state = fused && build_source;
+    if (!seed_state) TC_HIP_TRY(ctx, hipMemcpyAsync(ctx->state.p, hs, sizeof(IcpState), hipMemcpyHostToDevice, ctx->stream));
+    if (tc_status s = ensure(ctx, ctx->icp_wsrc, 2 * (ns + 4) * sizeof(float4))) return s;
     out.tg = plan_tiles((*out.tix).geom, ns);
     if (src_presorted && src_presorted->geom.n == ns) {
         out.src = (const float4 *)src_presorted->pts.p;
@@ -1666,6 +1669,8 @@
         IndexSpec source_order;
         source_order.reuse_geom = &(*out.tix).geom; source_order.state_transform = (const IcpState *)ctx->state.p;
         source_order.tile_major = &out.tg; source_order.strict_order = strict_source_order;
+        if (fused) source_order.working_copy = (float4 *)ctx->icp_wsrc.p;
+        if (seed_state) source_order.state_init = hs;
         if (ns > 0)
             if (tc_status s = build_index(ctx, ctx->src_index, d_src, ns, source_order)) return s;
         out.src = (const float4 *)ctx->src_index.pts.p;
@@ -1682,9 +1687,8 @@
         out.tix->pts12_valid = true;
     }
     out.tv = view_of((*out.tix));
-    if (tc_status s = ensure(ctx, ctx->icp_wsrc, 2 * (ns + 4) * sizeof(float4))) return s;
     out.wsrc = (float4 *)ctx->icp_wsrc.p;
-    if (ns > 0) {
+    if (ns > 0 && !(fused && build_source)) {
         ProfScope ps(ctx, "icp_working_source");
         hipLaunchKernelGGL(icp_working_source_kernel, dim3((unsigned)((ns + 255) / 256)), dim3(256), 0, ctx->stream, out.src, (uint32_t)ns, out.wsrc, (float4 *)nullptr);
     }
@@ -1811,7 +1815,7 @@
     const int mode = job.mode;
     const size_t ns = job.ns, nt = job.nt;
     IcpSetup su;
-    if (tc_status s = icp_setup(ctx, job, mode == 2 ? nullptr : job.src_presorted, false, su)) return s;
+    if (tc_status s = icp_setup(ctx, job, mode == 2 ? nullptr : job.src_presorted, false, true, su)) return s;
     su.wl = su.wsrc + ns + 4;
     hipStream_t st = ctx->stream;
     uint32_t *corr = (uint32_t *)ctx->corr.p, *corr_pos = match_words(su.wsrc);
@@ -1845,7 +1849,7 @@
     if (tc_status s = launch_finish(ctx, su, su.l.mse_blocks, 0, false, &hs)) return s;
     if (res->corr_target) {
         hipLaunchKernelGGL(icp_write_corr_kernel, dim3((unsigned)((ns + 255) / 256)), dim3(256), 0, st, su.tv, su.src, (uint32_t)ns,
-                           corr_pos, job.corr_on_device ? res->corr_target : corr);
+                           corr_pos, job.corr_on_device ? res->corr_target : corr, su.tix->orig_valid ? (const uint32_t *)su.tix->orig.p : nullptr);
         if (!job.corr_on_device) TC_HIP_TRY(ctx, hipMemcpyAsync(res->corr_target, corr, ns * sizeof(uint32_t), hipMemcpyDeviceToHost, st));
     }
     TC_HIP_TRY(ctx, hipStreamSynchronize(st));
@@ -1881,7 +1885,7 @@
     const size_t n_setup = ihi - ilo;
     IcpJob mine = job;
     mine.src = job.src + 3 * ilo; mine.ns = n_setup;
-    tc_status setup_rc = icp_setup(ctx, mine, nullptr, shard_mode == TC_SHARD_SPATIAL && W > 1, su);
+    tc_status setup_rc = icp_setup(ctx, mine, nullptr, shard_mode == TC_SHARD_SPATIAL && W > 1, false, su);
     if (setup_rc == TC_OK && !su.tix->vor_valid) setup_rc = ensure(ctx, su.tix->vor, (size_t)su.tix->geom.n * sizeof(float4));
     const bool gather_index = shard_mode == TC_SHARD_INDEX && res->corr_target && ns > 0 && (W > 1 || (comm && comm->nccl));
     if (setup_rc == TC_OK && gather_index) setup_rc = ensure(ctx, ctx->out_a, (size_t)W * rows * sizeof(uint32_t));
@@ -1916,14 +1920,15 @@
             uint32_t *all = (uint32_t *)ctx->out_a.p;
             if (nl > 0)
                 hipLaunchKernelGGL(icp_write_corr_kernel, dim3((unsigned)((nl + 255) / 256)), dim3(256), 0, st, su.tv, su.src, (uint32_t)nl, corr_pos,
-                                   all + (size_t)rank * rows);
+                                   all + (size_t)rank * rows, (const uint32_t *)nullptr);
             if (tc_status s = comm_allgather(comm, all, rows * sizeof(uint32_t))) return s;
             TC_HIP_TRY(ctx, hipMemcpyAsync(res->corr_target, all, ns * sizeof(uint32_t), hipMemcpyDeviceToDevice, st));
         } else {
             const bool gather = shard_mode == TC_SHARD_SPATIAL && (W > 1 || (comm && comm->nccl));
             if (gather) hipLaunchKernelGGL(icp_zero_u32_kernel, dim3((unsigned)((ns + 255) / 256)), dim3(256), 0, st, corr, (uint32_t)ns);
             if (nl > 0)
-                hipLaunchKernelGGL(icp_write_corr_kernel, dim3((unsigned)((nl + 255) / 256)), dim3(256), 0, st, su.tv, su.src, (uint32_t)nl, corr_pos, corr);
+                hipLaunchKernelGGL(icp_write_corr_kernel, dim3((unsigned)((nl + 255) / 256)), dim3(256), 0, st, su.tv, su.src, (uint32_t)nl, corr_pos, corr,
+                                   (const uint32_t *)nullptr);
             if (gather)
                 if (tc_status s = comm_allreduce_u32(comm, corr, ns)) return s;
             TC_HIP_TRY(ctx, hipMemcpyAsync(res->corr_target, corr, n_setup * sizeof(uint32_t), hipMemcpyDeviceToDevice, st));
@@ -1959,7 +1964,7 @@
     job.nrm = d_target_normals; job.nstride = normal_stride;
     job.init = init; job.max_dist = max_correspondence_distance; job.conv_thr = convergence_threshold;
     tc_icp_shard *s = new tc_icp_shard{ctx, {}};
-    tc_status rc = tc::icp_setup(ctx, job, nullptr, false, s->su);
+    tc_status rc = tc::icp_setup(ctx, job, nullptr, false, false, s->su);
     if (rc != TC_OK) { delete s; return rc; }
     *out = s;
     return TC_OK;
@@ -2011,7 +2016,7 @@
     if (res->corr_target) {
         uint32_t *corr = (uint32_t *)ctx->corr.p;
         hipLaunchKernelGGL(tc::icp_write_corr_kernel, dim3((unsigned)((su.ns + 255) / 256)), dim3(256), 0, st, su.tv, su.src, su.ns,
-                           tc::match_words(su.wsrc), corr);
+                           tc::match_words(su.wsrc), corr, (const uint32_t *)nullptr);
         TC_HIP_TRY(ctx, hipMemcpyAsync(res->corr_target, corr, su.ns * sizeof(uint32_t), hipMemcpyDeviceToDevice, st));
     }
     TC_HIP_TRY(ctx, hipStreamSynchronize(st));
diff --git a/threecrate_amd/csrc/tc_internal.h b/threecrate_amd/csrc/tc_internal.h
--- a/threecrate_amd/csrc/tc_internal.h
+++ b/threecrate_amd/csrc/tc_internal.h
@@ -297,6 +297,8 @@
     bool vor_valid = false;
     DevBuf pts12;
     bool pts12_valid = false;
+    DevBuf orig;
+    bool orig_valid = false;
     uint32_t occ_host = 0;
     bool occ_host_valid = false;
     DevBuf cell_of;
@@ -313,6 +315,20 @@
     const IcpState *state_transform = nullptr;
     const TileGeom *tile_major = nullptr;
     bool strict_order = false;
+    bool icp_target = false;
+    float4 *working_copy = nullptr;
+    const IcpState *state_init = nullptr;
+};
+struct PlaceExtras {
+    float    *pts12;
+    uint32_t *orig;
+    float4   *wsrc;
+};
+struct IcpSeed {
+    float   q[4], t[3];
+    float   conv_thr, max_dist;
+    int32_t kiss;
+    int32_t store;
 };
 __host__ __device__ inline int ball_rings(const GridGeom &g, float radius) {
     const int gyz = g.gy > g.gz ? g.gy : g.gz;
@@ -320,7 +336,7 @@
 }
 template <class F> void for_each_scratch_buf(DeviceIndex &ix, F f) { for (DevBuf *b : {&ix.cell_of, &ix.slot, &ix.arrival, &ix.fill, &ix.blocksum}) f(*b); }
 template <class F> void for_each_buf(DeviceIndex &ix, F f) {
-    for (DevBuf *b : {&ix.pts, &ix.cell_start, &ix.normals, &ix.vor, &ix.pts12}) f(*b);
+    for (DevBuf *b : {&ix.pts, &ix.cell_start, &ix.normals, &ix.vor, &ix.pts12, &ix.orig}) f(*b);
     for_each_scratch_buf(ix, f);
 }
 
```

New measurement: 18190 it/s, median of 6. Within noise of the previous version (+0.5%).
